# jinlinyi/PerspectiveFields

Hardware: NVIDIA H100
Metric: images/sec at 640x480 (Paramnet-360Cities-edina), H100 vs ref CPU (higher is better)
Workload: dtype f32 via 3x bf16 split MMA, fp32 accumulate

## Files before the change

### perspectivefields_b200/csrc/gemm_tma.cuh

```cuda
#pragma once
#include <cuda.h>

#include "tc_ptx.cuh"

namespace pf {

constexpr int MODE_GEMM = 0, MODE_HALO = 1;
constexpr int kTmaThreads = 384;
constexpr int kHaloBytes = 180 * 128;

struct TmaGemmParams {
  int M;
  int B, H, W;
  int Cin;
  int N, K;
  int a_c0, a_gc;
  int c_split, a2_c0;
  int groups;
  int b_row0;
  const float* bias; int bias_mode, bias_gstride;
  int act; const float* gamma;
  const float* res;  int ldr, r_coff, r_gcoff, res_relu;
  const float* res2; int ldr2, r2_coff, r2_gcoff;
  float* C; int ldc, c_coff, c_gcoff;
  __nv_bfloat16* Shi; __nv_bfloat16* Slo; int lds, s_coff, s_gcoff, split_relu;
  const float* pred_w; const float* pred_b; float* pred_out; int pred_nc, pred_mode;
  int phase4;
};

template <int BN, int MODE, int KB, bool PP = false, int NP = 3> struct TmaCfg {
  static_assert(KB == 32 || KB == 64, "KB");
  static_assert(BN % 32 == 0 && BN <= 256, "BN");
  static_assert(!PP || MODE == MODE_GEMM, "the ping-pong schedule is a GEMM-mode schedule");
  static_assert(NP == 1 || NP == 3, "NP");
  static constexpr int kPlanes = NP == 3 ? 2 : 1;
  static constexpr int kTileM = PP ? 64 : 128;
  static constexpr int kBPlane = BN * KB * 2;
  static constexpr int kAPlane = kTileM * KB * 2;
  static constexpr int kStage = (MODE == MODE_GEMM ? kPlanes * kAPlane : 0) + kPlanes * kBPlane;
  static constexpr int kABuf = kPlanes * kHtPlaneBytes;
  static constexpr int kAccPitch = 68;
  static constexpr int kAccStage = 2 * 64 * kAccPitch * 4;
  static constexpr int kBudget = 225 * 1024 - kAccStage - (MODE == MODE_HALO ? 2 * kABuf : 0);
  static constexpr int kStagesRaw = kBudget / kStage;
  static constexpr int kStages = kStagesRaw > 16 ? 16 : kStagesRaw;
  static constexpr int kSmemBytes = (MODE == MODE_HALO ? 2 * kABuf : 0) + kStages * kStage + kAccStage + 512 + 1024;
  static_assert(kStages >= 2, "ring too shallow");
  static_assert(kSmemBytes <= 227 * 1024, "shared memory per block");
};

__device__ __forceinline__ void mbar_expect_tx(uint32_t bar, uint32_t bytes) {
  asm volatile("mbarrier.arrive.expect_tx.shared::cta.b64 _, [%0], %1;\n" ::"r"(bar), "r"(bytes) : "memory");
}
__device__ __forceinline__ void tma_load_2d(uint32_t dst, const CUtensorMap* map, uint32_t bar, int c0, int c1) {
  asm volatile("cp.async.bulk.tensor.2d.shared::cluster.global.mbarrier::complete_tx::bytes [%0], [%1, {%3, %4}], [%2];\n"
               ::"r"(dst), "l"(reinterpret_cast<uint64_t>(map)), "r"(bar), "r"(c0), "r"(c1) : "memory");
}
__device__ __forceinline__ void tma_load_4d(uint32_t dst, const CUtensorMap* map, uint32_t bar, int c0, int c1, int c2, int c3) {
  asm volatile("cp.async.bulk.tensor.4d.shared::cluster.global.mbarrier::complete_tx::bytes [%0], [%1, {%3, %4, %5, %6}], [%2];\n"
               ::"r"(dst), "l"(reinterpret_cast<uint64_t>(map)), "r"(bar), "r"(c0), "r"(c1), "r"(c2), "r"(c3) : "memory");
}
__device__ __forceinline__ void tma_prefetch_desc(const CUtensorMap* map) {
  asm volatile("prefetch.tensormap [%0];\n" ::"l"(reinterpret_cast<uint64_t>(map)) : "memory");
}

struct TmaMaps {
  CUtensorMap a_hi, a_lo, a2_hi, a2_lo, b_hi, b_lo;
};

template <int BN, int MODE, int KB, bool PP = false, int NP = 3>
__global__ void __launch_bounds__(kTmaThreads, 1) gemm_tma_kernel(const __grid_constant__ TmaMaps maps, const TmaGemmParams p, int tiles_x, int tiles_y) {
  using Cfg = TmaCfg<BN, MODE, KB, PP, NP>;
  constexpr bool kLo = NP == 3;
  constexpr int NS = Cfg::kStages;
  constexpr int SPC = 9 * (64 / KB);
  constexpr int kConsumerWarps = PP ? 4 : 8;
  extern __shared__ unsigned char smem_dyn[];
  const uint32_t raw = smem_u32(smem_dyn);
  const uint32_t sbase = (raw + 1023u) & ~1023u;
  unsigned char* sm = smem_dyn + (sbase - raw);
  const uint32_t a_base = sbase;
  const uint32_t ring = sbase + (MODE == MODE_HALO ? 2 * Cfg::kABuf : 0);
  const uint32_t acc_base = ring + NS * Cfg::kStage;
  const uint32_t bars = acc_base + Cfg::kAccStage;
  auto full_b = [&](int s) { return bars + 8u * s; };
  auto empty_b = [&](int s) { return bars + 8u * (NS + s); };
  auto full_a = [&](int i) { return bars + 8u * (2 * NS + i); };
  auto empty_a = [&](int i) { return bars + 8u * (2 * NS + 2 + i); };
  auto order_b = [&](int w) { return bars + 8u * (2 * NS + 4 + w); };

  const int tid = threadIdx.x, lane = tid & 31, warp = tid >> 5;
  const int n_tiles = cdiv(p.N, BN);
  const int m_tiles = MODE == MODE_GEMM ? cdiv(p.M, Cfg::kTileM) : p.B * tiles_x * tiles_y;
  const int total_tiles = m_tiles * n_tiles * p.groups;
  const int nchunks = MODE == MODE_HALO ? p.Cin / 64 : 0;
  const int nk = MODE == MODE_GEMM ? p.K / KB : nchunks * SPC;
  const bool b_resident = MODE == MODE_HALO && nchunks == 1 && SPC <= NS;

  if (tid == 0) {
    tma_prefetch_desc(&maps.a_hi); tma_prefetch_desc(&maps.b_hi);
    if (kLo) { tma_prefetch_desc(&maps.a_lo); tma_prefetch_desc(&maps.b_lo); }
    for (int s = 0; s < NS; ++s) { mbar_init(full_b(s), 1); mbar_init(empty_b(s), kConsumerWarps); }
    for (int i = 0; i < 2; ++i) { mbar_init(full_a(i), 1); mbar_init(empty_a(i), kConsumerWarps); mbar_init(order_b(i), 4); }
    fence_mbar_init();
  }
  __syncthreads();
  pdl_wait();
  pdl_launch();

  auto decode = [&](int tile, int& mt, int& g, int& n0) {
    n0 = (tile % n_tiles) * BN;
    tile /= n_tiles;
    g = tile % p.groups;
    mt = tile / p.groups;
  };

  if (warp < 4) {
    asm volatile("setmaxnreg.dec.sync.aligned.u32 40;\n");
    if (warp == 0 && lane == 0) {
      int it = 0;
      for (int tile = blockIdx.x; tile < total_tiles; tile += gridDim.x) {
        int mt, g, n0;
        decode(tile, mt, g, n0);
        const int brow = p.b_row0 + g * p.N + n0;
        if (b_resident && it > 0) break;
        for (int kc = 0; kc < nk; ++kc, ++it) {
          const int s = it % NS;
          mbar_wait(empty_b(s), ((it / NS) & 1) ^ 1);
          mbar_expect_tx(full_b(s), Cfg::kStage);
          const uint32_t st = ring + s * Cfg::kStage;
          int kcol;
          if (MODE == MODE_GEMM) {
            kcol = kc * KB;
            tma_load_2d(st, &maps.a_hi, full_b(s), p.a_c0 + g * p.a_gc + kcol, mt * Cfg::kTileM);
            if (kLo) tma_load_2d(st + Cfg::kAPlane, &maps.a_lo, full_b(s), p.a_c0 + g * p.a_gc + kcol, mt * Cfg::kTileM);
          } else {
            const int c = kc / SPC, u = kc - c * SPC;
            kcol = KB == 32 ? (u >> 1) * p.Cin + c * 64 + (u & 1) * 32 : u * p.Cin + c * 64;
          }
          const uint32_t bdst = st + (MODE == MODE_GEMM ? Cfg::kPlanes * Cfg::kAPlane : 0);
          tma_load_2d(bdst, &maps.b_hi, full_b(s), kcol, brow);
          if (kLo) tma_load_2d(bdst + Cfg::kBPlane, &maps.b_lo, full_b(s), kcol, brow);
        }
      }
    } else if (MODE == MODE_HALO && warp == 1 && lane == 0) {
      int ita = 0;
      for (int tile = blockIdx.x; tile < total_tiles; tile += gridDim.x) {
        int mt, g, n0;
        decode(tile, mt, g, n0);
        const int tx = mt % tiles_x, ty = (mt / tiles_x) % tiles_y, bimg = mt / (tiles_x * tiles_y);
        for (int c = 0; c < nchunks; ++c, ++ita) {
          const int buf = ita & 1;
          mbar_wait(empty_a(buf), ((ita >> 1) & 1) ^ 1);
          mbar_expect_tx(full_a(buf), Cfg::kPlanes * kHaloBytes);
          const uint32_t dst = a_base + buf * Cfg::kABuf;
          const int ci = c * 64;
          if (p.c_split > 0 && ci >= p.c_split) {
            tma_load_4d(dst, &maps.a2_hi, full_a(buf), p.a2_c0 + ci - p.c_split, tx * kHtTileW - 1, ty * kHtTileH - 1, bimg);
            if (kLo) tma_load_4d(dst + kHtPlaneBytes, &maps.a2_lo, full_a(buf), p.a2_c0 + ci - p.c_split, tx * kHtTileW - 1, ty * kHtTileH - 1, bimg);
          } else {
            tma_load_4d(dst, &maps.a_hi, full_a(buf), p.a_c0 + g * p.a_gc + ci, tx * kHtTileW - 1, ty * kHtTileH - 1, bimg);
            if (kLo) tma_load_4d(dst + kHtPlaneBytes, &maps.a_lo, full_a(buf), p.a_c0 + g * p.a_gc + ci, tx * kHtTileW - 1, ty * kHtTileH - 1, bimg);
          }
        }
      }
    }
    return;
  }

  asm volatile("setmaxnreg.inc.sync.aligned.u32 232;\n");
  const int wg = (warp >> 2) - 1;
  const int wt = tid & 127;
  float* stage = reinterpret_cast<float*>(sm + (acc_base - sbase)) + wg * 64 * Cfg::kAccPitch;
  const int erow = wt & 63, eh = wt >> 6;
  const int r = PP ? erow : wg * 64 + erow;
  constexpr int kTileStep = PP ? 2 : 1;
  float acc[BN / 2];
  int it = 0, ita = 0;
  for (int tl = PP ? wg : 0, tile = blockIdx.x + tl * gridDim.x; tile < total_tiles; tile += kTileStep * gridDim.x, tl += kTileStep) {
    int mt, g, n0;
    decode(tile, mt, g, n0);
    if (PP) {
      it = tl * nk;
      if (tl > 0) mbar_wait(order_b(wg ^ 1), ((tl - 1) >> 1) & 1);
    }
    int prev_s = -1, prev_buf = -1;
    fence_regs(acc);
    for (int kc = 0; kc < nk; ++kc, ++it) {
      const int s = it % NS;
      uint32_t a_hi, a_lo;
      bool chunk_end = false;
      int buf = 0;
      if (MODE == MODE_HALO) {
        const int c = kc / SPC, u = kc - c * SPC;
        const int tap = KB == 32 ? (u >> 1) : u, ky = tap / 3, kx = tap - ky * 3;
        buf = ita & 1;
        if (u == 0) mbar_wait(full_a(buf), (ita >> 1) & 1);
        a_hi = a_base + buf * Cfg::kABuf + ((ky + 8 * wg) * kHtHaloW + kx) * 128 + (KB == 32 ? (u & 1) * 64 : 0);
        a_lo = a_hi + kHtPlaneBytes;
        chunk_end = u == SPC - 1;
      } else {
        a_hi = ring + s * Cfg::kStage + (PP ? 0 : wg * 64 * KB * 2);
        a_lo = a_hi + Cfg::kAPlane;
      }
      const int sb = b_resident ? kc : s;
      if (!b_resident || tl == 0) mbar_wait(full_b(sb), b_resident ? 0 : ((it / NS) & 1));
      const uint32_t b_hi = ring + sb * Cfg::kStage + (MODE == MODE_GEMM ? Cfg::kPlanes * Cfg::kAPlane : 0);
      const uint64_t dah = MODE == MODE_HALO ? ht_a_desc(a_hi) : wgmma_tile_desc<KB>(a_hi);
      const uint64_t dbh = wgmma_tile_desc<KB>(b_hi);
      wgmma_fence();
      if (kLo) {
        const uint64_t dal = MODE == MODE_HALO ? ht_a_desc(a_lo) : wgmma_tile_desc<KB>(a_lo);
        const uint64_t dbl = wgmma_tile_desc<KB>(b_hi + Cfg::kBPlane);
#pragma unroll
        for (int kk = 0; kk < KB / 16; ++kk) {
          const uint32_t first = (kc | kk) ? 1u : 0u;
          wgmma_bf16<BN>(acc, dal + 2 * kk, dbh + 2 * kk, first);
          wgmma_bf16<BN>(acc, dah + 2 * kk, dbl + 2 * kk, 1u);
          wgmma_bf16<BN>(acc, dah + 2 * kk, dbh + 2 * kk, 1u);
        }
      } else {
#pragma unroll
        for (int kk = 0; kk < KB / 16; ++kk) wgmma_bf16<BN>(acc, dah + 2 * kk, dbh + 2 * kk, (kc | kk) ? 1u : 0u);
      }
      wgmma_commit();
      wgmma_wait<1>();
      if (lane == 0 && prev_s >= 0) {
        if (!b_resident) mbar_arrive(empty_b(prev_s));
        if (MODE == MODE_HALO && prev_buf >= 0) mbar_arrive(empty_a(prev_buf));
      }
      prev_s = s;
      prev_buf = chunk_end ? buf : -1;
      if (MODE == MODE_HALO && chunk_end) ++ita;
    }
    if (PP && lane == 0) mbar_arrive(order_b(wg));
    wgmma_wait<0>();
    fence_regs(acc);
    if (lane == 0 && prev_s >= 0) {
      if (!b_resident) mbar_arrive(empty_b(prev_s));
      if (MODE == MODE_HALO && prev_buf >= 0) mbar_arrive(empty_a(prev_buf));
    }

    long long m;
    bool valid;
    int cls_off = 0;
    int bimg = 0, oy = 0, ox = 0;
    if (MODE == MODE_GEMM) {
      m = (long long)mt * Cfg::kTileM + r;
      valid = m < p.M;
    } else {
      const int tx = mt % tiles_x, ty = (mt / tiles_x) % tiles_y;
      bimg = mt / (tiles_x * tiles_y);
      oy = ty * kHtTileH + (r >> 3); ox = tx * kHtTileW + (r & 7);
      valid = oy < p.H && ox < p.W;
      m = ((long long)bimg * p.H + oy) * p.W + ox;
      if (p.bias_mode == 2) {
        const int ry = oy == 0 ? 0 : (oy == p.H - 1 ? 2 : 1);
        const int rx = ox == 0 ? 0 : (ox == p.W - 1 ? 2 : 1);
        cls_off = (ry * 3 + rx) * p.N;
      }
    }
    const float* __restrict__ bias = p.bias ? p.bias + (long long)g * p.bias_gstride : nullptr;
    const int frow = (wt >> 5) * 16 + (lane >> 2), fcol = 2 * (lane & 3);
#pragma unroll
    for (int rd = 0; rd < (BN + 63) / 64; ++rd) {
      named_bar_sync(1 + wg, 128);
#pragma unroll
      for (int jb = 0; jb < 8; ++jb) {
        const int cb = rd * 8 + jb;
        if (cb < BN / 8) {
          float* d0 = stage + frow * Cfg::kAccPitch + jb * 8 + fcol;
          *reinterpret_cast<float2*>(d0) = make_float2(acc[4 * cb], acc[4 * cb + 1]);
          *reinterpret_cast<float2*>(d0 + 8 * Cfg::kAccPitch) = make_float2(acc[4 * cb + 2], acc[4 * cb + 3]);
        }
      }
      named_bar_sync(1 + wg, 128);
      const int ch = 2 * rd + eh;
      const bool ph4 = MODE == MODE_HALO && BN == 128 && p.phase4;
      const bool staged_split = p.Shi && !ph4;
      float o[32];
      if (ch < BN / 32) {
        const int nb = n0 + ch * 32;
        const long long mo = ph4 ? ((long long)bimg * 2 * p.H + 2 * oy + (ch >> 1)) * (2 * p.W) + 2 * ox + (ch & 1) : m;
        const int nbo = ph4 ? 0 : nb;
        const bool chunk_ok = nb < p.N;
        const float* srow = stage + erow * Cfg::kAccPitch + eh * 32;
#pragma unroll
        for (int j = 0; j < 32; j += 4) {
          const float4 t = *reinterpret_cast<const float4*>(srow + j);
          o[j] = t.x; o[j + 1] = t.y; o[j + 2] = t.z; o[j + 3] = t.w;
        }
        if (valid && chunk_ok) {
          if (p.bias_mode) {
#pragma unroll
            for (int j = 0; j < 32; j += 4) {
              const float4 bv = __ldg(reinterpret_cast<const float4*>(bias + cls_off + nb + j));
              o[j] += bv.x; o[j + 1] += bv.y; o[j + 2] += bv.z; o[j + 3] += bv.w;
            }
          }
          if (p.act == 1) {
#pragma unroll
            for (int j = 0; j < 32; ++j) o[j] = fmaxf(o[j], 0.f);
          } else if (p.act == 2) {
#pragma unroll
            for (int j = 0; j < 32; ++j) o[j] = gelu_erf(o[j]);
          }
          if (p.gamma) {
#pragma unroll
            for (int j = 0; j < 32; j += 4) {
              const float4 gv = __ldg(reinterpret_cast<const float4*>(p.gamma + nb + j));
              o[j] *= gv.x; o[j + 1] *= gv.y; o[j + 2] *= gv.z; o[j + 3] *= gv.w;
            }
          }
          if (p.res) {
            const float* rp = p.res + m * p.ldr + p.r_coff + g * p.r_gcoff + nb;
#pragma unroll
            for (int j = 0; j < 32; j += 4) {
              float4 rv = *reinterpret_cast<const float4*>(rp + j);
              if (p.res_relu) { rv.x = fmaxf(rv.x, 0.f); rv.y = fmaxf(rv.y, 0.f); rv.z = fmaxf(rv.z, 0.f); rv.w = fmaxf(rv.w, 0.f); }
              o[j] += rv.x; o[j + 1] += rv.y; o[j + 2] += rv.z; o[j + 3] += rv.w;
            }
          }
          if (p.res2) {
            const float* rp = p.res2 + m * p.ldr2 + p.r2_coff + g * p.r2_gcoff + nb;
#pragma unroll
            for (int j = 0; j < 32; j += 4) {
              const float4 rv = *reinterpret_cast<const float4*>(rp + j);
              o[j] += rv.x; o[j + 1] += rv.y; o[j + 2] += rv.z; o[j + 3] += rv.w;
            }
          }
          if (MODE == MODE_HALO && (BN == 32 || BN == 128) && p.pred_w) {
            float v0 = __ldg(p.pred_b), v1 = p.pred_nc > 1 ? __ldg(p.pred_b + 1) : 0.f;
#pragma unroll
            for (int j = 0; j < 32; j += 4) {
              const float4 w0 = __ldg(reinterpret_cast<const float4*>(p.pred_w + j));
              v0 = fmaf(o[j], w0.x, v0); v0 = fmaf(o[j + 1], w0.y, v0); v0 = fmaf(o[j + 2], w0.z, v0); v0 = fmaf(o[j + 3], w0.w, v0);
              if (p.pred_nc > 1) {
                const float4 w1 = __ldg(reinterpret_cast<const float4*>(p.pred_w + 32 + j));
                v1 = fmaf(o[j], w1.x, v1); v1 = fmaf(o[j + 1], w1.y, v1); v1 = fmaf(o[j + 2], w1.z, v1); v1 = fmaf(o[j + 3], w1.w, v1);
              }
            }
            const long long HWl = (long long)p.H * p.W * (ph4 ? 4 : 1);
            const long long bi = mo / HWl, pix = mo - bi * HWl;
            float* po = p.pred_out + bi * p.pred_nc * HWl + pix;
            if (p.pred_mode == 1) {
              const float nrm = fmaxf(sqrtf(v0 * v0 + v1 * v1), 1e-12f);
              po[0] = v0 / nrm; po[HWl] = v1 / nrm;
            } else {
              po[0] = fminf(fmaxf(v0, -1.f), 1.f);
            }
          }
        }
        if (chunk_ok && (p.C || (p.Shi && !staged_split))) {
          const bool odd = lane & 1;
          const bool valid_p = __shfl_xor_sync(0xffffffffu, (int)valid, 1) != 0;
          const long long mo_p = mo + (odd ? -1 : 1) * (ph4 ? 2 : 1);
          const long long moA = odd ? mo_p : mo, moB = odd ? mo : mo_p;
          const bool vA = odd ? valid_p : valid, vB = odd ? valid : valid_p;
          if (p.C) {
            float* cA = p.C + moA * p.ldc + p.c_coff + g * p.c_gcoff + nbo + (odd ? 4 : 0);
            float* cB = p.C + moB * p.ldc + p.c_coff + g * p.c_gcoff + nbo + (odd ? 4 : 0);
#pragma unroll
            for (int t = 0; t < 4; ++t) {
              float k[4], rr[4];
#pragma unroll
              for (int e = 0; e < 4; ++e) {
                k[e] = odd ? o[8 * t + 4 + e] : o[8 * t + e];
                rr[e] = __shfl_xor_sync(0xffffffffu, odd ? o[8 * t + e] : o[8 * t + 4 + e], 1);
              }
              if (vA) *reinterpret_cast<float4*>(cA + 8 * t) = odd ? make_float4(rr[0], rr[1], rr[2], rr[3]) : make_float4(k[0], k[1], k[2], k[3]);
              if (vB) *reinterpret_cast<float4*>(cB + 8 * t) = odd ? make_float4(k[0], k[1], k[2], k[3]) : make_float4(rr[0], rr[1], rr[2], rr[3]);
            }
          }
          if (p.Shi && !staged_split) {
            const long long sA = moA * p.lds + p.s_coff + g * p.s_gcoff + nbo + (odd ? 8 : 0);
            const long long sB = moB * p.lds + p.s_coff + g * p.s_gcoff + nbo + (odd ? 8 : 0);
#pragma unroll
            for (int t = 0; t < 2; ++t) {
              float k[8], rr[8];
#pragma unroll
              for (int e = 0; e < 8; ++e) {
                const float mine = odd ? o[16 * t + 8 + e] : o[16 * t + e], give = odd ? o[16 * t + e] : o[16 * t + 8 + e];
                k[e] = p.split_relu ? fmaxf(mine, 0.f) : mine;
                rr[e] = __shfl_xor_sync(0xffffffffu, p.split_relu ? fmaxf(give, 0.f) : give, 1);
              }
              uint4 kh, kl, rh, rl;
              split_bf16x2(k[0], k[1], kh.x, kl.x); split_bf16x2(k[2], k[3], kh.y, kl.y);
              split_bf16x2(k[4], k[5], kh.z, kl.z); split_bf16x2(k[6], k[7], kh.w, kl.w);
              split_bf16x2(rr[0], rr[1], rh.x, rl.x); split_bf16x2(rr[2], rr[3], rh.y, rl.y);
              split_bf16x2(rr[4], rr[5], rh.z, rl.z); split_bf16x2(rr[6], rr[7], rh.w, rl.w);
              if (vA) {
                *reinterpret_cast<uint4*>(p.Shi + sA + 16 * t) = odd ? rh : kh;
                *reinterpret_cast<uint4*>(p.Slo + sA + 16 * t) = odd ? rl : kl;
              }
              if (vB) {
                *reinterpret_cast<uint4*>(p.Shi + sB + 16 * t) = odd ? kh : rh;
                *reinterpret_cast<uint4*>(p.Slo + sB + 16 * t) = odd ? kl : rl;
              }
            }
          }
        }
      }
      if (staged_split) {
        named_bar_sync(1 + wg, 128);
        unsigned char* sS = reinterpret_cast<unsigned char*>(stage);
        if (ch < BN / 32) {
#pragma unroll
          for (int t = 0; t < 4; ++t) {
            uint4 h, l;
            float k[8];
#pragma unroll
            for (int e = 0; e < 8; ++e) k[e] = p.split_relu ? fmaxf(o[8 * t + e], 0.f) : o[8 * t + e];
            split_bf16x2(k[0], k[1], h.x, l.x); split_bf16x2(k[2], k[3], h.y, l.y);
            split_bf16x2(k[4], k[5], h.z, l.z); split_bf16x2(k[6], k[7], h.w, l.w);
            const int off = erow * 128 + (((eh * 4 + t) ^ (erow & 7)) << 4);
            *reinterpret_cast<uint4*>(sS + off) = h;
            *reinterpret_cast<uint4*>(sS + 64 * 128 + off) = l;
          }
        }
        named_bar_sync(1 + wg, 128);
#pragma unroll
        for (int i = wt; i < 2 * 64 * 8; i += 128) {
          const int lo_plane = i >> 9, rr = (i >> 3) & 63, pc = i & 7;
          const int col = rd * 64 + pc * 8;
          if (col >= BN || n0 + col >= p.N) continue;
          long long mr;
          bool vr;
          if (MODE == MODE_GEMM) {
            mr = (long long)mt * Cfg::kTileM + (PP ? 0 : wg * 64) + rr;
            vr = mr < p.M;
          } else {
            const int rt = wg * 64 + rr, tx = mt % tiles_x, ty = (mt / tiles_x) % tiles_y;
            const int py = ty * kHtTileH + (rt >> 3), px = tx * kHtTileW + (rt & 7);
            vr = py < p.H && px < p.W;
            mr = ((long long)bimg * p.H + py) * p.W + px;
          }
          if (!vr) continue;
          const uint4 v = *reinterpret_cast<const uint4*>(sS + lo_plane * 64 * 128 + rr * 128 + ((pc ^ (rr & 7)) << 4));
          *reinterpret_cast<uint4*>((lo_plane ? p.Slo : p.Shi) + mr * p.lds + p.s_coff + g * p.s_gcoff + n0 + col) = v;
        }
      }
    }
  }
}

}
```

### perspectivefields_b200/csrc/pf_b200.cu

```cuda
#include "../../include/pf_b200.h"

#include <cuda_runtime.h>
#include <nvtx3/nvToolsExt.h>

#include <atomic>
#include <cctype>
#include <cmath>
#include <cstdarg>
#include <cstdio>
#include <cstdlib>
#include <cstring>
#include <map>
#include <mutex>
#include <string>
#include <functional>
#include <unordered_map>
#include <vector>

#include "common.cuh"
#include "tma_host.cuh"
#include "attention_mma.cuh"
#include "layers.cuh"
#include "prepost.cuh"
#include "pano.cuh"
#include "comm.cuh"
#include "jpeg.cuh"

using namespace pf;

static thread_local std::string g_err;
static std::atomic<long long> g_launches{0};

static int fail(int code, const char* fmt, ...) {
  char buf[1024];
  va_list ap;
  va_start(ap, fmt);
  vsnprintf(buf, sizeof(buf), fmt, ap);
  va_end(ap);
  g_err = buf;
  return code;
}
#define CU(expr)                                                                                    \
  do {                                                                                              \
    cudaError_t e__ = (expr);                                                                       \
    if (e__ != cudaSuccess) return fail(PF_ERR_CUDA, "%s: %s (%s:%d)", #expr, cudaGetErrorString(e__), __FILE__, __LINE__); \
  } while (0)
static char g_crumb[96] = "";
static bool sync_debug() {
  static int v = -1;
  if (v < 0) v = getenv("PF_SYNC_DEBUG") ? 1 : 0;
  return v == 1;
}
struct KernelProf {
  bool on = false;
  cudaStream_t st = nullptr;
  std::vector<cudaEvent_t> pool;
  size_t used = 0;
  struct Rec { const char* expr; cudaEvent_t a, b; };
  std::vector<Rec> recs;
  cudaEvent_t next() { return used < pool.size() ? pool[used++] : nullptr; }
};
static thread_local KernelProf* tl_kp = nullptr;
#define LAUNCHED(expr)                                                                              \
  do {                                                                                              \
    KernelProf* kp__ = tl_kp;                                                                       \
    cudaEvent_t ka__ = (kp__ && kp__->on) ? kp__->next() : nullptr;                                 \
    if (ka__) cudaEventRecord(ka__, kp__->st);                                                      \
    cudaError_t e__ = (expr);                                                                       \
    g_launches.fetch_add(1, std::memory_order_relaxed);                                             \
    if (ka__) {                                                                                     \
      cudaEvent_t kb__ = kp__->next();                                                              \
      if (kb__) { cudaEventRecord(kb__, kp__->st); kp__->recs.push_back({#expr, ka__, kb__}); }     \
    }                                                                                               \
    if (e__ == cudaSuccess && sync_debug()) e__ = cudaDeviceSynchronize();                          \
    if (e__ != cudaSuccess) return fail(PF_ERR_CUDA, "%s: %s (%s:%d, after tap '%s')", #expr, cudaGetErrorString(e__), __FILE__, __LINE__, g_crumb); \
  } while (0)
struct NvtxRange {
  explicit NvtxRange(const char* name) { nvtxRangePushA(name); }
  ~NvtxRange() { nvtxRangePop(); }
};
#define TRY(expr)                \
  do {                           \
    int r__ = (expr);            \
    if (r__ != PF_OK) return r__; \
  } while (0)

static const int kMitDims[4] = {64, 128, 320, 512};
static const int kMitHeads[4] = {1, 2, 5, 8};
static const int kMitDepths[4] = {3, 4, 18, 3};
static const int kMitSr[4] = {8, 4, 2, 1};
static const int kCnxDims[4] = {96, 192, 384, 768};
static const int kCnxDepths[4] = {3, 3, 9, 3};

struct WeightRef { const void* p; long long numel; int dtype; };
struct GemmW { const __nv_bfloat16* hi = nullptr; const __nv_bfloat16* lo = nullptr; const float* b = nullptr; };
struct LnW { const float* w = nullptr; const float* b = nullptr; };

struct MitBlockW { LnW ln1, srln, ln2; GemmW q, sr, kv, proj, fc1, fc2; const float* dw_w; const float* dw_b; };
struct CnxBlockW { const float* dw_w; const float* dw_b; LnW ln; GemmW pw1, pw2; const float* gamma; };

struct Arena {
  char* base = nullptr;
  long long cap = 0, off = 0, peak = 0;
  bool dry = false, keep = false;
  void* alloc(long long bytes) {
    off = (off + 255) & ~255LL;
    void* p = dry ? nullptr : base + off;
    off += bytes;
    if (off > peak) peak = off;
    return p;
  }
  float* f(long long n) { return (float*)alloc(n * 4); }
  long long mark() const { return off; }
  void release(long long m) { if (!keep) off = m; }
};

struct pf_engine {
  int device = 0;
  pf_model_desc desc{};
  int net_h = kNet, net_w = kNet;
  bool finalized = false;
  std::unordered_map<std::string, WeightRef> weights;
  const float *embed1_w, *embed1_b, *llenc_w, *llenc_b;
  LnW embed_ln[4], stage_norm[4];
  GemmW embed[4];
  GemmW embed1g, llencg;
  std::vector<MitBlockW> blocks[4];
  GemmW proc[4];
  GemmW rcu[4][2][2];
  GemmW conv0, conv1;
  GemmW conv1p;
  const float *conv1f_w, *conv1f_b;
  bool use_fork = false;
  cudaStream_t side = nullptr;
  cudaEvent_t ev_fork = nullptr, ev_join = nullptr;
  bool use_dwln = false;
  bool use_pdl = true;
  bool decode_only = false;
  bool use_attn_split = true;
  bool use_phase = true;
  const float *pred_g_w, *pred_g_b, *pred_l_w, *pred_l_b;
  const float *pn_stem_w, *pn_stem_b;
  LnW pn_stem_ln, pn_ds_ln[4], pn_norm;
  GemmW pn_ds[4];
  std::vector<CnxBlockW> pn_blocks[4];
  const float *pn_head_w, *pn_head_b;
  struct DevTable { int ksize; int* bounds; int* coeffs; };
  std::map<std::pair<int, int>, DevTable> tables;
  char* table_dev = nullptr;
  char* table_host = nullptr;
  long long table_off = 0;
  KernelProf kp;
  struct MapKey {
    const void* base; long long d0, d1, d2; int kind, box, kb;
    bool operator==(const MapKey& o) const { return base == o.base && d0 == o.d0 && d1 == o.d1 && d2 == o.d2 && kind == o.kind && box == o.box && kb == o.kb; }
  };
  struct MapKeyHash {
    size_t operator()(const MapKey& k) const {
      size_t h = std::hash<const void*>()(k.base);
      for (long long v : {k.d0, k.d1, k.d2, (long long)k.kind, (long long)k.box, (long long)k.kb}) h = h * 1000003u ^ std::hash<long long>()(v);
      return h;
    }
  };
  std::unordered_map<MapKey, CUtensorMap, MapKeyHash> map_cache;
  bool use_stem_tc = true;
  bool use_attn_mma = true;
  bool bf16 = false;
  int sm_count = 132;
  bool profile = false;
  struct ProfRec { cudaEvent_t a, b; double flops; int cfg; int M, N, K, KH, stride, groups, Cin; };
  std::vector<ProfRec> prof;
  std::vector<cudaEvent_t> ev_pool;
  bool debug = false;
  std::vector<std::pair<std::string, std::pair<const float*, long long>>> taps;
};

static int get_w(pf_engine* e, const std::string& name, int dtype, long long numel, const void** out) {
  auto it = e->weights.find(name);
  if (it == e->weights.end()) return fail(PF_ERR_WEIGHT, "missing weight '%s'", name.c_str());
  if (it->second.dtype != dtype) return fail(PF_ERR_WEIGHT, "weight '%s': wrong dtype", name.c_str());
  if (it->second.numel != numel) return fail(PF_ERR_WEIGHT, "weight '%s': numel %lld, expected %lld", name.c_str(), it->second.numel, numel);
  *out = it->second.p;
  return PF_OK;
}
static int get_f(pf_engine* e, const std::string& n, long long numel, const float** out) { return get_w(e, n, PF_F32, numel, (const void**)out); }
static int get_gemm(pf_engine* e, const std::string& n, long long N, long long K, long long nbias, GemmW* g, int groups = 1) {
  TRY(get_w(e, n + ".whi", PF_BF16, groups * N * K, (const void**)&g->hi));
  TRY(get_w(e, n + ".wlo", PF_BF16, groups * N * K, (const void**)&g->lo));
  TRY(get_f(e, n + ".b", groups * nbias, &g->b));
  return PF_OK;
}
static int get_ln(pf_engine* e, const std::string& n, int C, LnW* l) {
  TRY(get_f(e, n + ".w", C, &l->w));
  TRY(get_f(e, n + ".b", C, &l->b));
  return PF_OK;
}

static int resolve_weights(pf_engine* e) {
  char nm[128];
  TRY(get_f(e, "embed1.w", 147 * 64, &e->embed1_w));
  TRY(get_f(e, "embed1.b", 64, &e->embed1_b));
  TRY(get_f(e, "llenc.w", 147 * 64, &e->llenc_w));
  TRY(get_f(e, "llenc.b", 64, &e->llenc_b));
  TRY(get_gemm(e, "embed1g", 64, 160, 64, &e->embed1g));
  TRY(get_gemm(e, "llencg", 64, 160, 64, &e->llencg));
  for (int s = 0; s < 4; ++s) {
    const int C = kMitDims[s];
    snprintf(nm, sizeof nm, "embed%d.ln", s + 1);
    TRY(get_ln(e, nm, C, &e->embed_ln[s]));
    if (s > 0) {
      snprintf(nm, sizeof nm, "embed%d", s + 1);
      TRY(get_gemm(e, nm, C, 9LL * kMitDims[s - 1], C, &e->embed[s]));
    }
    e->blocks[s].resize(kMitDepths[s]);
    for (int i = 0; i < kMitDepths[s]; ++i) {
      MitBlockW& b = e->blocks[s][i];
      char p[64];
      snprintf(p, sizeof p, "s%d.b%d.", s + 1, i);
      std::string P(p);
      TRY(get_ln(e, P + "ln1", C, &b.ln1));
      TRY(get_gemm(e, P + "q", C, C, C, &b.q));
      if (kMitSr[s] > 1) {
        TRY(get_gemm(e, P + "sr", C, (long long)kMitSr[s] * kMitSr[s] * C, C, &b.sr));
        TRY(get_ln(e, P + "srln", C, &b.srln));
      }
      TRY(get_gemm(e, P + "kv", 2 * C, C, 2 * C, &b.kv));
      TRY(get_gemm(e, P + "proj", C, C, C, &b.proj));
      TRY(get_ln(e, P + "ln2", C, &b.ln2));
      TRY(get_gemm(e, P + "fc1", 4 * C, C, 4 * C, &b.fc1));
      TRY(get_f(e, P + "dw.w", 9LL * 4 * C, &b.dw_w));
      TRY(get_f(e, P + "dw.b", 4 * C, &b.dw_b));
      TRY(get_gemm(e, P + "fc2", C, 4 * C, C, &b.fc2));
    }
    snprintf(nm, sizeof nm, "s%d.norm", s + 1);
    TRY(get_ln(e, nm, C, &e->stage_norm[s]));
  }
  for (int l = 0; l < 4; ++l) {
    snprintf(nm, sizeof nm, "head.proc%d", l + 1);
    TRY(get_gemm(e, nm, 512, 9LL * kMitDims[l], 9 * 512, &e->proc[l]));
  }
  for (int f = 0; f < 4; ++f)
    for (int u = 0; u < 2; ++u) {
      if (f == 3 && u == 0) continue;
      for (int c = 0; c < 2; ++c) {
        snprintf(nm, sizeof nm, "head.f%d.u%d.c%d", f + 1, u + 1, c + 1);
        TRY(get_gemm(e, nm, 256, 2304, 256, &e->rcu[f][u][c], 2));
      }
    }
  TRY(get_gemm(e, "head.conv0", 64, 9 * 320, 64, &e->conv0, 2));
  TRY(get_gemm(e, "head.conv1", 32, 9 * 64, 32, &e->conv1, 2));
  TRY(get_gemm(e, "head.conv1p", 128, 9 * 64, 128, &e->conv1p, 2));
  TRY(get_f(e, "head.conv1f.w", 2LL * 9 * 64 * 32, &e->conv1f_w));
  TRY(get_f(e, "head.conv1f.b", 64, &e->conv1f_b));
  TRY(get_f(e, "head.pred_g.w", 32LL * e->desc.gravity_classes, &e->pred_g_w));
  TRY(get_f(e, "head.pred_g.b", e->desc.gravity_classes, &e->pred_g_b));
  TRY(get_f(e, "head.pred_l.w", 32LL * e->desc.latitude_classes, &e->pred_l_w));
  TRY(get_f(e, "head.pred_l.b", e->desc.latitude_classes, &e->pred_l_b));
  if (e->desc.param_net != PF_PARAM_NONE) {
    TRY(get_f(e, "pn.stem.w", 48 * 96, &e->pn_stem_w));
    TRY(get_f(e, "pn.stem.b", 96, &e->pn_stem_b));
    TRY(get_ln(e, "pn.stem.ln", 96, &e->pn_stem_ln));
    for (int k = 1; k < 4; ++k) {
      snprintf(nm, sizeof nm, "pn.ds%d.ln", k);
      TRY(get_ln(e, nm, kCnxDims[k - 1], &e->pn_ds_ln[k]));
      snprintf(nm, sizeof nm, "pn.ds%d", k);
      TRY(get_gemm(e, nm, kCnxDims[k], 4LL * kCnxDims[k - 1], kCnxDims[k], &e->pn_ds[k]));
    }
    for (int s = 0; s < 4; ++s) {
      const int C = kCnxDims[s];
      e->pn_blocks[s].resize(kCnxDepths[s]);
      for (int j = 0; j < kCnxDepths[s]; ++j) {
        CnxBlockW& b = e->pn_blocks[s][j];
        char p[64];
        snprintf(p, sizeof p, "pn.s%d.b%d.", s, j);
        std::string P(p);
        TRY(get_f(e, P + "dw.w", 49LL * C, &b.dw_w));
        TRY(get_f(e, P + "dw.b", C, &b.dw_b));
        TRY(get_ln(e, P + "ln", C, &b.ln));
        TRY(get_gemm(e, P + "pw1", 4 * C, C, 4 * C, &b.pw1));
        TRY(get_gemm(e, P + "pw2", C, 4 * C, C, &b.pw2));
        TRY(get_f(e, P + "gamma", C, &b.gamma));
      }
    }
    TRY(get_ln(e, "pn.norm", 768, &e->pn_norm));
    TRY(get_f(e, "pn.head.w", 5 * 768, &e->pn_head_w));
    TRY(get_f(e, "pn.head.b", 5, &e->pn_head_b));
  }
  return PF_OK;
}

struct Fwd {
  pf_engine* e;
  Arena ar;
  cudaStream_t st;
  bool dry;
  int n;

  int tap(const char* name, const float* p, long long numel) {
    if (!e->debug) return PF_OK;
    float* cp = ar.f(numel);
    if (dry) return PF_OK;
    snprintf(g_crumb, sizeof g_crumb, "%s", name);
    if (sync_debug()) fprintf(stderr, "[pf tap] %s cp=%p (+%lld of cap %lld) p=%p numel=%lld\n", name, (void*)cp, (long long)((char*)cp - ar.base), ar.cap, (const void*)p, numel);
    CU(cudaMemcpyAsync(cp, p, numel * 4, cudaMemcpyDeviceToDevice, st));
    if (sync_debug()) CU(cudaDeviceSynchronize());
    e->taps.push_back({name, {cp, numel}});
    return PF_OK;
  }
  int tapf(const float* p, long long numel, const char* fmt, ...) {
    if (!e->debug) return PF_OK;
    char buf[96];
    va_list ap;
    va_start(ap, fmt);
    vsnprintf(buf, sizeof buf, fmt, ap);
    va_end(ap);
    return tap(buf, p, numel);
  }

  SplitT salloc(long long pixels, int ld) {
    SplitT t;
    t.hi = (__nv_bfloat16*)ar.alloc(pixels * ld * 2);
    t.lo = (__nv_bfloat16*)ar.alloc(pixels * ld * 2);
    t.ld = ld;
    return t;
  }
  int tap_split(const char* name, const SplitT& t, long long numel) {
    if (!e->debug) return PF_OK;
    float* cp = ar.f(numel);
    if (dry) return PF_OK;
    snprintf(g_crumb, sizeof g_crumb, "%s", name);
    LAUNCHED((merge_split_kernel<<<(unsigned)cdivl(numel, 256), 256, 0, st>>>(t.hi, t.lo, cp, numel), cudaGetLastError()));
    e->taps.push_back({name, {cp, numel}});
    return PF_OK;
  }
  static cudaError_t gemm_tma_gemm_mode(const TmaMaps& maps, const TmaGemmParams& p, int bn, int kb, bool pp, int np, int sms, cudaStream_t st, const PredTail* pred) {
    return gemm_tma_launch(MODE_GEMM, maps, p, bn, kb, pp, np, sms, st, pred);
  }
  static cudaError_t gemm_tma_halo_mode(const TmaMaps& maps, const TmaGemmParams& p, int bn, int kb, bool pp, int np, int sms, cudaStream_t st, const PredTail* pred) {
    return gemm_tma_launch(MODE_HALO, maps, p, bn, kb, pp, np, sms, st, pred);
  }
  int np() const { return e->bf16 ? 1 : 3; }
  int force_bn = 0, force_kb = 0;
  int force_sched = 0;
  int picked_bn = 0, picked_kb = 0, picked_sched = 0;
  int pick_tile(int mode, const TmaGemmParams& p, const PredTail* pred, int& bn, int& kb, bool& pp) {
    tma_pick_tile(mode, p.M, p.N, p.K, e->sm_count, bn, kb);
    if (force_bn) { bn = force_bn; kb = tma_pick_kb(bn, p.K, mode); }
    if (force_kb) kb = force_kb;
    pp = mode == MODE_GEMM && (force_sched ? force_sched == 2 : tma_pick_pingpong(p.M, p.N, p.K, bn, e->sm_count));
    if (const char* msg = gemm_tma_check(mode, p, bn, kb, pred != nullptr, pp, np())) return fail(PF_ERR_ARG, "TMA engine, %s (bn %d, kb %d): %s", mode == MODE_GEMM ? "GEMM mode" : "halo mode", bn, kb, msg);
    picked_bn = bn; picked_kb = kb; picked_sched = mode == MODE_GEMM ? (pp ? 2 : 1) : 0;
    return PF_OK;
  }
  int launch_tma(int mode, const TmaMaps& maps, const TmaGemmParams& p, int bn, int kb, bool pp, const PredTail* pred = nullptr) {
    if (e->profile) {
      pf_engine::ProfRec r{};
      for (cudaEvent_t* ev : {&r.a, &r.b}) {
        if (e->ev_pool.empty()) { CU(cudaEventCreate(ev)); }
        else { *ev = e->ev_pool.back(); e->ev_pool.pop_back(); }
      }
      const double Mrows = mode == MODE_GEMM ? (double)p.M : (double)p.B * p.H * p.W;
      r.flops = 2.0 * Mrows * (double)p.N * (double)p.K * (double)p.groups;
      r.cfg = mode == MODE_GEMM ? 5 : 6;
      r.M = (int)Mrows; r.N = p.N; r.K = p.K; r.KH = mode == MODE_GEMM ? 1 : 3; r.stride = 1; r.groups = p.groups; r.Cin = p.Cin;
      CU(cudaEventRecord(r.a, st));
      if (mode == MODE_GEMM) LAUNCHED(gemm_tma_gemm_mode(maps, p, bn, kb, pp, np(), e->sm_count, st, pred));
      else LAUNCHED(gemm_tma_halo_mode(maps, p, bn, kb, pp, np(), e->sm_count, st, pred));
      CU(cudaEventRecord(r.b, st));
      e->prof.push_back(r);
      return PF_OK;
    }
    if (mode == MODE_GEMM) LAUNCHED(gemm_tma_gemm_mode(maps, p, bn, kb, pp, np(), e->sm_count, st, pred));
    else LAUNCHED(gemm_tma_halo_mode(maps, p, bn, kb, pp, np(), e->sm_count, st, pred));
    return PF_OK;
  }
  struct Epi {
    float* C = nullptr; int ldc = 0, c_coff = 0, c_gcoff = 0;
    SplitT S; int s_coff = 0, s_gcoff = 0, split_relu = 0;
    int act = 0; const float* gamma = nullptr;
    const float* res = nullptr; int ldr = 0, r_coff = 0, r_gcoff = 0, res_relu = 0;
    const float* res2 = nullptr; int ldr2 = 0, r2_coff = 0, r2_gcoff = 0;
    int bias_mode = 1;
    int phase4 = 0;
  };
  static void fill_epi(TmaGemmParams& p, const GemmW& w, const Epi& o, int bias_gstride) {
    p.bias = w.b; p.bias_mode = w.b ? o.bias_mode : 0; p.bias_gstride = bias_gstride;
    p.act = o.act; p.gamma = o.gamma;
    p.res = o.res; p.ldr = o.ldr; p.r_coff = o.r_coff; p.r_gcoff = o.r_gcoff; p.res_relu = o.res_relu;
    p.res2 = o.res2; p.ldr2 = o.ldr2; p.r2_coff = o.r2_coff; p.r2_gcoff = o.r2_gcoff;
    p.C = o.C; p.ldc = o.ldc; p.c_coff = o.c_coff; p.c_gcoff = o.c_gcoff;
    p.Shi = o.S.hi; p.Slo = o.S.lo; p.lds = o.S.ld; p.s_coff = o.s_coff; p.s_gcoff = o.s_gcoff; p.split_relu = o.split_relu;
    p.phase4 = o.phase4;
  }
  template <class F>
  const char* cached_map(CUtensorMap* out, const pf_engine::MapKey& key, F&& make) {
    auto it = e->map_cache.find(key);
    if (it != e->map_cache.end()) { *out = it->second; return nullptr; }
    const char* msg = make(out);
    if (!msg) {
      if (e->map_cache.size() > 20000) e->map_cache.clear();
      e->map_cache.emplace(key, *out);
    }
    return msg;
  }
  const char* map2d(CUtensorMap* m, const void* base, long long cols, long long rows, long long ld, int box_rows, int kb) {
    return cached_map(m, pf_engine::MapKey{base, cols, rows, ld, 0, box_rows, kb}, [&](CUtensorMap* o) { return tma_map_2d(o, base, cols, rows, ld, box_rows, kb); });
  }
  const char* map_halo(CUtensorMap* m, const void* base, int B, int H, int W, int ld) {
    return cached_map(m, pf_engine::MapKey{base, ((long long)B << 32) | (unsigned)H, W, ld, 3, 0, 0}, [&](CUtensorMap* o) { return tma_map_halo(o, base, B, H, W, ld); });
  }
  int tgemm(const SplitT& A, long long M, int K, int a_c0, const GemmW& w, int N, const Epi& o) {
    if (dry) return PF_OK;
    if (K % 32 || N % 32 || A.ld % 8) return fail(PF_ERR_ARG, "tgemm: K/N must be multiples of 32");
    if (o.res2 || o.bias_mode == 2) return fail(PF_ERR_ARG, "tgemm: second residual / border-class bias are halo-mode features");
    TmaGemmParams p{};
    p.M = (int)M; p.Cin = K; p.N = N; p.K = K; p.a_c0 = a_c0; p.groups = 1;
    fill_epi(p, w, o, 0);
    TmaMaps maps{};
    int bn, kb;
    bool pp;
    TRY(pick_tile(MODE_GEMM, p, nullptr, bn, kb, pp));
    const char* msg = nullptr;
    const int a_rows = pp ? 64 : 128;
    if (!msg) msg = map2d(&maps.a_hi, A.hi, A.ld, M, A.ld, a_rows, kb);
    if (!msg) msg = map2d(&maps.a_lo, A.lo, A.ld, M, A.ld, a_rows, kb);
    if (!msg) msg = map2d(&maps.b_hi, w.hi, K, N, K, bn, kb);
    if (!msg) msg = map2d(&maps.b_lo, w.lo, K, N, K, bn, kb);
    if (msg) return fail(PF_ERR_CUDA, "%s", msg);
    maps.a2_hi = maps.a_hi; maps.a2_lo = maps.a_lo;
    return launch_tma(MODE_GEMM, maps, p, bn, kb, pp);
  }
  int thalo(const SplitT& A, int a_c0, int a_gc, const SplitT* A2, int c_split, int a2_c0, int B, int H, int W, int Cin, const GemmW& w, int N,
            int groups, int bias_gstride, const Epi& o, const PredTail* pred = nullptr) {
    if (dry) return PF_OK;
    if (Cin % 64 || N % 32 || (A2 && c_split % 64)) return fail(PF_ERR_ARG, "thalo: Cin must be a multiple of 64, N of 32");
    if (w.b && o.bias_mode == 2 && (H < 2 || W < 2)) return fail(PF_ERR_ARG, "thalo: border-class bias needs H, W >= 2 (got %dx%d)", H, W);
    TmaGemmParams p{};
    p.B = B; p.H = H; p.W = W; p.Cin = Cin; p.N = N; p.K = 9 * Cin; p.a_c0 = a_c0; p.a_gc = a_gc; p.groups = groups;
    p.c_split = A2 ? c_split : 0; p.a2_c0 = a2_c0;
    fill_epi(p, w, o, bias_gstride);
    TmaMaps maps{};
    int bn, kb;
    bool pp;
    TRY(pick_tile(MODE_HALO, p, pred, bn, kb, pp));
    const char* msg = nullptr;
    if (!msg) msg = map_halo(&maps.a_hi, A.hi, B, H, W, A.ld);
    if (!msg) msg = map_halo(&maps.a_lo, A.lo, B, H, W, A.ld);
    if (A2) {
      if (!msg) msg = map_halo(&maps.a2_hi, A2->hi, B, H, W, A2->ld);
      if (!msg) msg = map_halo(&maps.a2_lo, A2->lo, B, H, W, A2->ld);
    } else { maps.a2_hi = maps.a_hi; maps.a2_lo = maps.a_lo; }
    if (!msg) msg = map2d(&maps.b_hi, w.hi, p.K, (long long)groups * N, p.K, bn, kb);
    if (!msg) msg = map2d(&maps.b_lo, w.lo, p.K, (long long)groups * N, p.K, bn, kb);
    if (msg) return fail(PF_ERR_CUDA, "%s", msg);
    return launch_tma(MODE_HALO, maps, p, bn, kb, pp, pred);
  }
  int tconv_gather(const SplitT& A, int B, int H, int W, int Cin, int KH, int stride, int pad, const GemmW& w, int N, const Epi& o) {
    const int OH = (H + 2 * pad - KH) / stride + 1, OW = (W + 2 * pad - KH) / stride + 1;
    const long long M = (long long)B * OH * OW;
    const int K = KH * KH * Cin;
    const long long m = ar.mark();
    SplitT col = salloc(M, K);
    if (!dry) {
      if (Cin % 8) return fail(PF_ERR_ARG, "tconv_gather: Cin %% 8");
      LAUNCHED(launch_pdl(im2col_split_kernel, dim3(ew_grid(M * K / 8)), dim3(256), 0, st, A.hi, A.lo, A.ld, col.hi, col.lo, B, H, W, Cin, OH, OW, KH, stride, pad));
    }
    int r = tgemm(col, M, K, 0, w, N, o);
    ar.release(m);
    return r;
  }
  int ln_split(const float* x, const SplitT& y, long long rows, int C, const LnW& w, float eps, float* yf = nullptr) {
    if (dry) return PF_OK;
    LAUNCHED(layernorm_launch(x, yf, rows, C, w.w, w.b, eps, st, y));
    return PF_OK;
  }
  int ln_split_patch(const float* x, const SplitT& y, const SplitT& patch, long long rows, int C, const LnW& w, float eps, int RH, int RW, int sr) {
    if (dry) return PF_OK;
    LAUNCHED(layernorm_launch(x, nullptr, rows, C, w.w, w.b, eps, st, y, patch, RH, RW, sr));
    return PF_OK;
  }
  int ln(const float* x, float* y, long long rows, int C, const LnW& w, float eps) {
    if (dry) return PF_OK;
    LAUNCHED(layernorm_launch(x, y, rows, C, w.w, w.b, eps, st));
    return PF_OK;
  }
};

constexpr long long kTableSlabBytes = 8LL << 20;
static int get_table(pf_engine* e, int in_size, int out_size, pf_engine::DevTable* out, cudaStream_t st) {
  auto it = e->tables.find({in_size, out_size});
  if (it == e->tables.end()) {
    ResampleTable t = make_resample_table(in_size, out_size);
    const long long nb = (long long)t.bounds.size() * sizeof(int), nc = (long long)t.coeffs.size() * sizeof(int);
    const long long need = ((nb + 255) & ~255LL) + ((nc + 255) & ~255LL);
    if (need > kTableSlabBytes) return fail(PF_ERR_ARG, "image axis of %d pixels is too long for the resize tables", in_size);
    if (e->table_off + need > kTableSlabBytes) {
      CU(cudaStreamSynchronize(st));
      e->tables.clear();
      e->table_off = 0;
    }
    pf_engine::DevTable d{};
    d.ksize = t.ksize;
    const long long o0 = e->table_off, o1 = o0 + ((nb + 255) & ~255LL);
    memcpy(e->table_host + o0, t.bounds.data(), nb);
    memcpy(e->table_host + o1, t.coeffs.data(), nc);
    d.bounds = (int*)(e->table_dev + o0);
    d.coeffs = (int*)(e->table_dev + o1);
    CU(cudaMemcpyAsync(e->table_dev + o0, e->table_host + o0, need, cudaMemcpyHostToDevice, st));
    e->table_off += need;
    it = e->tables.emplace(std::make_pair(in_size, out_size), d).first;
  }
  *out = it->second;
  return PF_OK;
}

static int pre_rows_needed(int H, int OH) {
  const double scale = (double)H / OH;
  const double support = scale < 1.0 ? 1.0 : scale;
  return (int)(kPreRows * scale) + 2 * (int)ceil(support) + 3;
}
static int pre_max_smem_rows(int OW) { return kPreSmemBytes / (OW * 3); }

static int fwd_preprocess(Fwd& F, const pf_batch* bt, float*& x0, PreImage*& d_pre, PostImage*& d_post) {
  pf_engine* e = F.e;
  const pf_model_desc& D = e->desc;
  const int n = F.n;
  const bool dry = F.dry;
  cudaStream_t st = F.st;
  Arena& ar = F.ar;
  const int NH = e->net_h, NW = e->net_w;
  const int max_rows = pre_max_smem_rows(NW);
  x0 = ar.f((long long)n * NH * NW * 4);
  d_pre = (PreImage*)ar.alloc((long long)n * sizeof(PreImage));
  d_post = (PostImage*)ar.alloc((long long)n * sizeof(PostImage));
  if (!dry) {
    if (bt->images_u8) {
      std::vector<PreImage> pre(n);
      int max_h = 1;
      for (int i = 0; i < n; ++i) {
        const int H = bt->height[i], W = bt->width[i];
        if (H < 1 || W < 1) return fail(PF_ERR_ARG, "image %d has size %dx%d", i, H, W);
        pf_engine::DevTable tx, ty;
        TRY(get_table(e, W, NW, &tx, st));
        TRY(get_table(e, H, NH, &ty, st));
        if (ty.ksize + 1 > max_rows) return fail(PF_ERR_ARG, "image %d is too tall (%d rows) for the resize kernel", i, H);
        pre[i] = PreImage{bt->image_offset[i], H, W, tx.ksize, ty.ksize, tx.bounds, tx.coeffs, ty.bounds, ty.coeffs};
        if (H > max_h) max_h = H;
      }
      CU(cudaMemcpyAsync(d_pre, pre.data(), n * sizeof(PreImage), cudaMemcpyHostToDevice, st));
      int rows = pre_rows_needed(max_h, NH);
      if (rows > max_rows) rows = max_rows;
      const int smem = rows * NW * 3;
      LAUNCHED((preprocess_kernel<<<dim3(NH / kPreRows, n), NW, smem, st>>>(bt->images_u8, d_pre, x0, D.pixel_mean[0], D.pixel_mean[1],
                                                                           D.pixel_mean[2], D.pixel_std[0], D.pixel_std[1], D.pixel_std[2], rows, NH, NW),
                cudaGetLastError()));
    } else {
      const long long total = (long long)n * NH * NW;
      LAUNCHED((normalize_chw_kernel<<<(unsigned)cdivl(total, 256), 256, 0, st>>>(bt->images_chw, x0, n, NH, NW, D.pixel_mean[0], D.pixel_mean[1],
                                                                                 D.pixel_mean[2], D.pixel_std[0], D.pixel_std[1], D.pixel_std[2]),
                cudaGetLastError()));
    }
  }
  return PF_OK;
}

static int launch_postprocess(const float* vec, const float* lat, int n, int SH, int SW, const int32_t* height, const int32_t* width, const int64_t* g_off,
                              const int64_t* l_off, float* g_out, float* l_out, int lat_is_sin, PostImage* d_post, cudaStream_t st) {
  std::vector<PostImage> post(n);
  long long total = 0;
  int max_h = 1, max_wp = 4;
  for (int i = 0; i < n; ++i) {
    if (height[i] < 1 || width[i] < 1) return fail(PF_ERR_ARG, "image %d has size %dx%d", i, height[i], width[i]);
    post[i] = PostImage{height[i], width[i], g_off[i], l_off[i], total};
    total += (long long)height[i] * width[i];
    if (height[i] > max_h) max_h = height[i];
    const int wp = (width[i] + 3) / 4 * 4;
    if (wp <= kPostMaxW && wp > max_wp) max_wp = wp;
  }
  CU(cudaMemcpyAsync(d_post, post.data(), n * sizeof(PostImage), cudaMemcpyHostToDevice, st));
  const int smem = post_smem_bytes(SW, max_wp);
  LAUNCHED((postprocess_kernel<<<dim3((unsigned)cdiv(max_h, kPostBand), (unsigned)n), kPostThreads, smem, st>>>(vec, lat, d_post, g_out, l_out, lat_is_sin, SH, SW),
            cudaGetLastError()));
  return PF_OK;
}

static int fwd_tails_post(Fwd& F, const pf_batch* bt, const float* conv1_out, PostImage* d_post, bool pred_done = false) {
  pf_engine* e = F.e;
  const pf_model_desc& D = e->desc;
  const int n = F.n;
  const bool dry = F.dry;
  cudaStream_t st = F.st;
  Arena& ar = F.ar;
  const int HW = e->net_h * e->net_w;
  const bool cls_g = D.gravity_classes != 2, cls_l = D.latitude_classes != 1;
  const bool fused_decode = e->decode_only && (cls_g || cls_l);
  if (e->decode_only && cls_g != cls_l) return fail(PF_ERR_ARG, "decode_only needs both heads to be classification heads");
  const float* vec = dry ? nullptr : bt->pred_gravity;
  const float* lat = dry ? nullptr : bt->pred_latitude;
  if (e->debug) {
    float* rg = ar.f((long long)n * D.gravity_classes * HW);
    float* rl = ar.f((long long)n * D.latitude_classes * HW);
    if (!dry) {
      const unsigned grid = (unsigned)cdivl((long long)n * HW, 128);
      LAUNCHED((pred_tail_kernel<<<grid, 128, D.gravity_classes * 33 * 4, st>>>(conv1_out, 64, 0, e->pred_g_w, e->pred_g_b, rg, n, HW, D.gravity_classes, 0), cudaGetLastError()));
      LAUNCHED((pred_tail_kernel<<<grid, 128, D.latitude_classes * 33 * 4, st>>>(conv1_out, 64, 32, e->pred_l_w, e->pred_l_b, rl, n, HW, D.latitude_classes, 0), cudaGetLastError()));
    }
    TRY(F.tap("head.raw_g", rg, (long long)n * D.gravity_classes * HW));
    TRY(F.tap("head.raw_l", rl, (long long)n * D.latitude_classes * HW));
  }
  if (fused_decode) {
    if (!dry) {
      const unsigned grid = ew_grid((long long)n * HW * 4);
      LAUNCHED((pred_argmax_decode_kernel<<<grid, 256, D.gravity_classes * 37 * 4, st>>>(conv1_out, 64, 0, e->pred_g_w, e->pred_g_b, bt->pred_gravity, n, HW,
                                                                                      D.gravity_classes, 1), cudaGetLastError()));
      LAUNCHED((pred_argmax_decode_kernel<<<grid, 256, D.latitude_classes * 37 * 4, st>>>(conv1_out, 64, 32, e->pred_l_w, e->pred_l_b, bt->pred_latitude, n, HW,
                                                                                       D.latitude_classes, 0), cudaGetLastError()));
    }
  } else {
    if (!dry && !pred_done) {
      const unsigned grid = (unsigned)cdivl((long long)n * HW, 128);
      LAUNCHED((pred_tail_kernel<<<grid, 128, D.gravity_classes * 33 * 4, st>>>(conv1_out, 64, 0, e->pred_g_w, e->pred_g_b, bt->pred_gravity, n, HW,
                                                                             D.gravity_classes, D.gravity_classes == 2 ? 1 : 0), cudaGetLastError()));
      LAUNCHED((pred_tail_kernel<<<grid, 128, D.latitude_classes * 33 * 4, st>>>(conv1_out, 64, 32, e->pred_l_w, e->pred_l_b, bt->pred_latitude, n, HW,
                                                                              D.latitude_classes, D.latitude_classes == 1 ? 2 : 0), cudaGetLastError()));
    }
    if (cls_g) {
      float* dv = ar.f((long long)n * 2 * HW);
      if (!dry) LAUNCHED((argmax_decode_kernel<<<(unsigned)cdivl((long long)n * HW, 256), 256, 0, st>>>(bt->pred_gravity, dv, n, HW, D.gravity_classes, 1), cudaGetLastError()));
      vec = dv;
    }
    if (cls_l) {
      float* dl = ar.f((long long)n * HW);
      if (!dry) LAUNCHED((argmax_decode_kernel<<<(unsigned)cdivl((long long)n * HW, 256), 256, 0, st>>>(bt->pred_latitude, dl, n, HW, D.latitude_classes, 0), cudaGetLastError()));
      lat = dl;
    }
  }
  if (!dry)
    TRY(launch_postprocess(vec, lat, n, e->net_h, e->net_w, bt->height, bt->width, bt->gravity_original_offset, bt->latitude_original_offset, bt->gravity_original,
                           bt->latitude_original, cls_l ? 0 : 1, d_post, st));
  return PF_OK;
}

static int run_forward_tma(Fwd& F, const pf_batch* bt) {
  pf_engine* e = F.e;
  const pf_model_desc& D = e->desc;
  const int n = F.n;
  const bool dry = F.dry;
  cudaStream_t st = F.st;
  Arena& ar = F.ar;
  using Epi = Fwd::Epi;
  const int NH = e->net_h, NW = e->net_w;
  int RH[4], RW[4];
  for (int s = 0; s < 4; ++s) { RH[s] = NH >> (s + 2); RW[s] = NW >> (s + 2); }
  const int nkv = RH[3] * RW[3];
  if ((NH != kNet || NW != kNet) && (!e->use_attn_mma || !e->use_attn_split || !e->use_stem_tc || !e->use_phase))
    return fail(PF_ERR_ARG, "options attn_mma / attn_split / stem_tc / phase_conv1 = 0 (reference paths of the 320 x 320 graph) need a 320 x 320 "
                            "working size; this engine runs at %d x %d", NH, NW);

  float* x0; PreImage* d_pre; PostImage* d_post;
  {
    NvtxRange r_("pf:preprocess");
    TRY(fwd_preprocess(F, bt, x0, d_pre, d_post));
  }
  TRY(F.tap("pre", x0, (long long)n * NH * NW * 4));

  NvtxRange* sect = new NvtxRange("pf:ll_enc");
  struct SectGuard { NvtxRange*& p; ~SectGuard() { delete p; } } sect_guard{sect};
  auto section = [&](const char* name) { delete sect; sect = nullptr; sect = new NvtxRange(name); };
  SplitT cfeat[4];
  for (int s = 0; s < 4; ++s) cfeat[s] = F.salloc((long long)n * RH[s] * RW[s], kMitDims[s]);
  const int LH = NH / 2, LW = NW / 2;
  SplitT ll = F.salloc((long long)n * LH * LW, 64);
  if (e->use_stem_tc) {
    const long long m = ar.mark();
    const long long M = (long long)n * LH * LW;
    SplitT col = F.salloc(M, 160);
    if (!dry) LAUNCHED(launch_pdl(stem_gather_kernel, dim3(ew_grid(stem_gather_threads(n, LH, LW))), dim3(256), 0, st, x0, col.hi, col.lo, n, LH, LW, 2, NH, NW));
    Epi o; o.S = ll; o.act = 1;
    TRY(F.tgemm(col, M, 160, 0, e->llencg, 64, o));
    ar.release(m);
  } else if (!dry) {
    LAUNCHED((stem_conv_launch<7, 7, 2, 3, 64>(x0, 4, n, kNet, kNet, e->llenc_w, e->llenc_b, nullptr, 1, st, ll)));
  }
  TRY(F.tap_split("ll", ll, (long long)n * LH * LW * 64));

  for (int s = 0; s < 4; ++s) {
    { char nm[32]; snprintf(nm, sizeof nm, "pf:mit.stage%d", s + 1); section(nm); }
    const int C = kMitDims[s], N = RH[s] * RW[s], heads = kMitHeads[s], sr = kMitSr[s];
    const long long rows = (long long)n * N;
    const long long m = ar.mark();
    float* x = ar.f(rows * C);
    float* tf = ar.f(rows * C);
    SplitT t1 = F.salloc(rows, C);
    SplitT t1p;
    if (sr > 1) t1p = F.salloc((long long)n * nkv, sr * sr * C);
    SplitT q = F.salloc(rows, C);
    SplitT a = F.salloc(rows, C);
    float* t2f = ar.f((long long)n * nkv * C);
    SplitT t2 = F.salloc((long long)n * nkv, C);
    SplitT kv = F.salloc((long long)n * nkv, 2 * C);
    const bool qkv_split = e->use_attn_mma && e->use_attn_split;
    float* qf = qkv_split ? nullptr : ar.f(rows * C);
    float* kvf = qkv_split ? nullptr : ar.f((long long)n * nkv * 2 * C);
    float* h1 = ar.f(rows * 4 * C);
    SplitT h2 = F.salloc(rows, 4 * C);
    if (s == 0 && e->use_stem_tc) {
      const long long mm = ar.mark();
      SplitT col = F.salloc(rows, 160);
      if (!dry) LAUNCHED(launch_pdl(stem_gather_kernel, dim3(ew_grid(stem_gather_threads(n, RH[0], RW[0]))), dim3(256), 0, st, x0, col.hi, col.lo, n, RH[0], RW[0], 4, NH, NW));
      Epi o; o.C = tf; o.ldc = C;
      TRY(F.tgemm(col, rows, 160, 0, e->embed1g, 64, o));
      ar.release(mm);
    } else if (s == 0) {
      if (!dry) LAUNCHED((stem_conv_launch<7, 7, 4, 3, 64>(x0, 4, n, kNet, kNet, e->embed1_w, e->embed1_b, tf, 0, st)));
    } else {
      Epi o; o.C = tf; o.ldc = C;
      TRY(F.tconv_gather(cfeat[s - 1], n, RH[s - 1], RW[s - 1], kMitDims[s - 1], 3, 2, 1, e->embed[s], C, o));
    }
    TRY(F.ln(tf, x, rows, C, e->embed_ln[s], 1e-5f));
    TRY(F.tapf(x, rows * C, "mit.s%d.embed", s + 1));
    for (int i = 0; i < kMitDepths[s]; ++i) {
      const MitBlockW& b = e->blocks[s][i];
      if (sr > 1) TRY(F.ln_split_patch(x, t1, t1p, rows, C, b.ln1, 1e-6f, RH[s], RW[s], sr));
      else TRY(F.ln_split(x, t1, rows, C, b.ln1, 1e-6f));
      Epi oq, okv;
      if (qkv_split) { oq.S = q; okv.S = kv; } else { oq.C = qf; oq.ldc = C; okv.C = kvf; okv.ldc = 2 * C; }
      const bool fork = !dry && sr > 1 && e->use_fork && e->side && !e->kp.on && !e->profile && !sync_debug() && !e->debug;
      if (fork) {
        CU(cudaEventRecord(e->ev_fork, st));
        CU(cudaStreamWaitEvent(e->side, e->ev_fork, 0));
        F.st = e->side;
      }
      if (sr > 1) {
        { Epi o; o.C = t2f; o.ldc = C; TRY(F.tgemm(t1p, (long long)n * nkv, sr * sr * C, 0, b.sr, C, o)); }
        TRY(F.ln_split(t2f, t2, (long long)n * nkv, C, b.srln, 1e-5f));
        TRY(F.tgemm(t2, (long long)n * nkv, C, 0, b.kv, 2 * C, okv));
      }
      if (fork) {
        CU(cudaEventRecord(e->ev_join, e->side));
        F.st = st;
      }
      TRY(F.tgemm(t1, rows, C, 0, b.q, C, oq));
      if (fork) CU(cudaStreamWaitEvent(st, e->ev_join, 0));
      if (sr > 1) {
      } else {
        TRY(F.tgemm(t1, rows, C, 0, b.kv, 2 * C, okv));
      }
      if (!dry) {
        if (qkv_split) LAUNCHED(attention_mma_launch(nullptr, nullptr, nullptr, n, N, C, heads, st, a, q, kv, F.np(), nkv));
        else if (e->use_attn_mma) LAUNCHED(attention_mma_launch(qf, kvf, nullptr, n, N, C, heads, st, a, SplitT(), SplitT(), F.np()));
        else LAUNCHED(attention_launch(qf, kvf, nullptr, n, N, C, heads, st, a));
      }
      { Epi o; o.C = x; o.ldc = C; o.res = x; o.ldr = C; TRY(F.tgemm(a, rows, C, 0, b.proj, C, o)); }
      TRY(F.tapf(x, rows * C, "mit.s%d.b%d.attn", s + 1, i));
      TRY(F.ln_split(x, t1, rows, C, b.ln2, 1e-6f));
      { Epi o; o.C = h1; o.ldc = 4 * C; TRY(F.tgemm(t1, rows, C, 0, b.fc1, 4 * C, o)); }
      if (!dry) LAUNCHED(launch_pdl(dwconv3x3_gelu_kernel, dim3(ew_grid((long long)n * ((RH[s] + 1) / 2) * ((RW[s] + PF_DW3_PX - 1) / PF_DW3_PX) * C)), dim3(256), 0, st, h1, nullptr, n, RH[s], RW[s], 4 * C, b.dw_w, b.dw_b, h2.hi, h2.lo));
      { Epi o; o.C = x; o.ldc = C; o.res = x; o.ldr = C; TRY(F.tgemm(h2, rows, 4 * C, 0, b.fc2, C, o)); }
      TRY(F.tapf(x, rows * C, "mit.s%d.b%d", s + 1, i));
    }
    TRY(F.ln_split(x, cfeat[s], rows, C, e->stage_norm[s], 1e-6f));
    { char nm[32]; snprintf(nm, sizeof nm, "mit.c%d", s + 1); TRY(F.tap_split(nm, cfeat[s], rows * C)); }
    ar.release(m);
  }

  float* conv1_out = ar.f((long long)n * NH * NW * 64);
  bool fuse_pred = false;
  {
    const long long m = ar.mark();
    float* fused = nullptr;
    SplitT fused_s;
    for (int lvl = 4; lvl >= 1; --lvl) {
      { char nm[32]; snprintf(nm, sizeof nm, "pf:heads.level%d", lvl); section(nm); }
      const int rh = RH[lvl - 1], rw = RW[lvl - 1], Cin = kMitDims[lvl - 1];
      const long long px = (long long)n * rh * rw;
      float* t = ar.f(px * 512);
      SplitT rt = F.salloc(px, 512);
      SplitT u = F.salloc(px, 512);
      float* v = ar.f(px * 512);
      SplitT rv = F.salloc(px, 512);
      float* w2 = ar.f(px * 512);
      {
        Epi o; o.C = t; o.ldc = 512; o.S = rt; o.split_relu = 1; o.bias_mode = 2;
        TRY(F.thalo(cfeat[lvl - 1], 0, 0, nullptr, 0, 0, n, rh, rw, Cin, e->proc[lvl - 1], 512, 1, 0, o));
        TRY(F.tapf(t, px * 512, "head.proc%d", lvl));
      }
      auto rcu = [&](const SplitT& A, const GemmW& w, Epi o) {
        o.c_gcoff = 256; o.s_gcoff = 256; o.r_gcoff = 256; o.r2_gcoff = 256;
        return F.thalo(A, 0, 256, nullptr, 0, 0, n, rh, rw, 256, w, 256, 2, 256, o);
      };
      const float* of = t;
      const SplitT* os = &rt;
      if (lvl < 4) {
        { Epi o; o.S = u; o.act = 1; TRY(rcu(rt, e->rcu[lvl - 1][0][0], o)); }
        { Epi o; o.C = v; o.ldc = 512; o.S = rv; o.split_relu = 1; o.res = t; o.ldr = 512; o.res_relu = 1; o.res2 = fused; o.ldr2 = 512;
          TRY(rcu(u, e->rcu[lvl - 1][0][1], o)); }
        of = v; os = &rv;
      }
      { Epi o; o.S = u; o.act = 1; TRY(rcu(*os, e->rcu[lvl - 1][1][0], o)); }
      { Epi o; o.C = w2; o.ldc = 512; o.res = of; o.ldr = 512; o.res_relu = 1; TRY(rcu(u, e->rcu[lvl - 1][1][1], o)); }
      if (lvl > 1) {
        float* up = ar.f(px * 4 * 512);
        if (!dry) LAUNCHED(launch_pdl(upsample2x_kernel, dim3(ew_grid(upsample2x_threads(n, rh, rw, 512))), dim3(256), 0, st, w2, 512, 0, up, 512, 0, n, rh, rw, 512, nullptr, nullptr));
        fused = up;
        TRY(F.tapf(up, px * 4 * 512, "head.fusion%d", lvl));
      } else {
        fused_s = F.salloc(px * 4, 512);
        if (!dry) LAUNCHED(launch_pdl(upsample2x_kernel, dim3(ew_grid(upsample2x_threads(n, rh, rw, 512))), dim3(256), 0, st, w2, 512, 0, nullptr, 512, 0, n, rh, rw, 512, fused_s.hi, fused_s.lo));
        TRY(F.tap_split("head.fusion1", fused_s, px * 4 * 512));
      }
    }
    section("pf:heads.fuse_convs");
    fuse_pred = D.gravity_classes == 2 && D.latitude_classes == 1;
    const bool keep_conv1 = !fuse_pred || e->debug;
    PredTail pt[2] = {{e->pred_g_w, e->pred_g_b, dry ? nullptr : bt->pred_gravity, 2, 1}, {e->pred_l_w, e->pred_l_b, dry ? nullptr : bt->pred_latitude, 1, 2}};
    if (e->use_phase) {
      SplitT c0s = F.salloc((long long)n * LH * LW, 128);
      {
        Epi o; o.S = c0s; o.s_gcoff = 64; o.act = 1;
        TRY(F.thalo(fused_s, 0, 256, &ll, 256, 0, n, LH, LW, 320, e->conv0, 64, 2, 64, o));
        TRY(F.tap_split("head.conv0", c0s, (long long)n * LH * LW * 128));
      }
      Epi o; o.ldc = 64; o.c_gcoff = 32; o.act = 1; o.phase4 = 1;
      if (keep_conv1) o.C = conv1_out;
      TRY(F.thalo(c0s, 0, 64, nullptr, 0, 0, n, LH, LW, 64, e->conv1p, 128, 2, 128, o, fuse_pred ? pt : nullptr));
      if (!dry) {
        const dim3 grid((unsigned)cdiv(conv1_ring_count(NH, NW), kRingPx), (unsigned)n);
        LAUNCHED((conv1_ring_kernel<<<grid, 256, kRingSmem, st>>>(c0s.hi, c0s.lo, LH, LW, e->conv1f_w, e->conv1f_b, keep_conv1 ? conv1_out : nullptr,
                                                                 fuse_pred ? e->pred_g_w : nullptr, e->pred_g_b, bt->pred_gravity,
                                                                 fuse_pred ? e->pred_l_w : nullptr, e->pred_l_b, bt->pred_latitude), cudaGetLastError()));
      }
    } else {
      float* c0 = ar.f((long long)n * 160 * 160 * 128);
      {
        Epi o; o.C = c0; o.ldc = 128; o.c_gcoff = 64; o.act = 1;
        TRY(F.thalo(fused_s, 0, 256, &ll, 256, 0, n, 160, 160, 320, e->conv0, 64, 2, 64, o));
        TRY(F.tap("head.conv0", c0, (long long)n * 160 * 160 * 128));
      }
      SplitT c0u = F.salloc((long long)n * kNet * kNet, 128);
      if (!dry) LAUNCHED(launch_pdl(upsample2x_kernel, dim3(ew_grid(upsample2x_threads(n, 160, 160, 128))), dim3(256), 0, st, c0, 128, 0, nullptr, 128, 0, n, 160, 160, 128, c0u.hi, c0u.lo));
      Epi o; o.ldc = 64; o.c_gcoff = 32; o.act = 1;
      if (keep_conv1) o.C = conv1_out;
      TRY(F.thalo(c0u, 0, 64, nullptr, 0, 0, n, kNet, kNet, 64, e->conv1, 32, 2, 32, o, fuse_pred ? pt : nullptr));
    }
    if (keep_conv1) TRY(F.tap("head.conv1", conv1_out, (long long)n * NH * NW * 64));
    ar.release(m);
  }
  section("pf:tails_postprocess");
  TRY(fwd_tails_post(F, bt, conv1_out, d_post, fuse_pred));

  if (D.param_net != PF_PARAM_NONE) {
    section("pf:paramnet");
    if (D.gravity_classes != 2 || D.latitude_classes != 1) return fail(PF_ERR_ARG, "ParamNet needs regression heads");
    const bool centered = D.param_net == PF_PARAM_CENTERED;
    const int SH = centered ? NH : D.param_input_size, SW = centered ? NW : D.param_input_size;
    float* pin = ar.f((long long)n * SH * SW * 4);
    if (!dry) LAUNCHED((pack_fields_kernel<<<(unsigned)cdivl((long long)n * SH * SW, 256), 256, 0, st>>>(bt->pred_gravity, bt->pred_latitude, pin, n, NH, NW, SH, SW), cudaGetLastError()));
    int rh = SH / 4, rw = SW / 4;
    float* x = ar.f((long long)n * rh * rw * 96);
    if (!dry) LAUNCHED((stem_conv_launch<4, 4, 4, 0, 96>(pin, 4, n, SH, SW, e->pn_stem_w, e->pn_stem_b, x, 0, st)));
    TRY(F.ln(x, x, (long long)n * rh * rw, 96, e->pn_stem_ln, 1e-6f));
    for (int s = 0; s < 4; ++s) {
      const int C = kCnxDims[s];
      if (s > 0) {
        const int r2h = rh / 2, r2w = rw / 2;
        SplitT y = F.salloc((long long)n * r2h * r2w, 4 * kCnxDims[s - 1]);
        TRY(F.ln_split_patch(x, SplitT(), y, (long long)n * rh * rw, kCnxDims[s - 1], e->pn_ds_ln[s], 1e-6f, rh, rw, 2));
        float* xn = ar.f((long long)n * r2h * r2w * C);
        Epi o; o.C = xn; o.ldc = C;
        TRY(F.tgemm(y, (long long)n * r2h * r2w, 4 * kCnxDims[s - 1], 0, e->pn_ds[s], C, o));
        x = xn; rh = r2h; rw = r2w;
      }
      const long long rows = (long long)n * rh * rw;
      float* yf = ar.f(rows * C);
      SplitT y = F.salloc(rows, C);
      SplitT h = F.salloc(rows, 4 * C);
      for (int j = 0; j < kCnxDepths[s]; ++j) {
        const CnxBlockW& b = e->pn_blocks[s][j];
        if (e->use_dwln) {
          if (!dry) LAUNCHED(dwconv7x7_ln_launch(x, n, rh, rw, C, b.dw_w, b.dw_b, b.ln.w, b.ln.b, 1e-6f, y, st));
        } else {
          if (!dry) LAUNCHED(launch_pdl(dwconv7x7_kernel, dim3(ew_grid((long long)n * ((rh + 1) / 2) * ((rw + PF_DW7_PX - 1) / PF_DW7_PX) * (C / 4))), dim3(256), 0, st, x, yf, n, rh, rw, C, b.dw_w, b.dw_b));
          TRY(F.ln_split(yf, y, rows, C, b.ln, 1e-6f));
        }
        { Epi o; o.S = h; o.act = 2; TRY(F.tgemm(y, rows, C, 0, b.pw1, 4 * C, o)); }
        { Epi o; o.C = x; o.ldc = C; o.res = x; o.ldr = C; o.gamma = b.gamma; TRY(F.tgemm(h, rows, 4 * C, 0, b.pw2, C, o)); }
      }
      TRY(F.tapf(x, rows * C, "cnx.s%d", s));
    }
    if (!dry) {
      if (!bt->params) return fail(PF_ERR_ARG, "params output is NULL");
      LAUNCHED((param_tail_kernel<<<n, 256, 0, st>>>(x, rh * rw, e->pn_norm.w, e->pn_norm.b, e->pn_head_w, e->pn_head_b, bt->params, D.param_net), cudaGetLastError()));
    }
  }
  return PF_OK;
}

extern "C" {

int pf_abi_version(void) { return PF_ABI_VERSION; }
const char* pf_last_error(void) { return g_err.c_str(); }
int64_t pf_kernel_launch_count(void) { return g_launches.load(); }

static int configure_device(int device) {
  static std::mutex mu;
  static std::vector<char> done;
  std::lock_guard<std::mutex> lock(mu);
  if (device < (int)done.size() && done[device]) return PF_OK;
  CU(gemm_tma_configure_device(3));
  CU(gemm_tma_configure_device(1));
  CU(attention_mma_configure_device());
  CU(cudaFuncSetAttribute(attention_kernel, cudaFuncAttributeMaxDynamicSharedMemorySize, kAttnSmem));
  CU(cudaFuncSetAttribute(conv1_ring_kernel, cudaFuncAttributeMaxDynamicSharedMemorySize, kRingSmem));
  CU(cudaFuncSetAttribute(preprocess_kernel, cudaFuncAttributeMaxDynamicSharedMemorySize, kPreSmemBytes));
  CU(cudaFuncSetAttribute(postprocess_kernel, cudaFuncAttributeMaxDynamicSharedMemorySize, kPostSmemMax));
  if (device >= (int)done.size()) done.resize(device + 1, 0);
  done[device] = 1;
  return PF_OK;
}
static int configure_current_device() {
  int dev = 0;
  CU(cudaGetDevice(&dev));
  return configure_device(dev);
}

static bool net_size_ok(int h, int w) {
  return h >= 64 && w >= 64 && h <= 640 && w <= 640 && h % 32 == 0 && w % 32 == 0 && (h / 32) * (w / 32) <= kAmMaxKeys;
}

int pf_create(int device, const pf_model_desc* desc, pf_handle* out) { return pf_create_sized(device, desc, kNet, kNet, out); }

int pf_create_sized(int device, const pf_model_desc* desc, int net_h, int net_w, pf_handle* out) {
  if (!desc || !out) return fail(PF_ERR_ARG, "pf_create: null argument");
  if (!net_size_ok(net_h, net_w))
    return fail(PF_ERR_ARG, "pf_create: working size %dx%d: height and width must be multiples of 32 in [64, 640] with (H/32)*(W/32) <= %d", net_h, net_w, kAmMaxKeys);
  if (!((desc->gravity_classes == 2 || desc->gravity_classes == 73) && (desc->latitude_classes == 1 || desc->latitude_classes == 180)))
    return fail(PF_ERR_ARG, "pf_create: unsupported head widths %d/%d", desc->gravity_classes, desc->latitude_classes);
  if (desc->param_net < 0 || desc->param_net > 2) return fail(PF_ERR_ARG, "pf_create: bad param_net");
  if (desc->param_net == PF_PARAM_UNCENTERED && (desc->param_input_size < 32 || desc->param_input_size > kNet || desc->param_input_size % 32))
    return fail(PF_ERR_ARG, "pf_create: param_input_size must be a multiple of 32 in [32, 320]");
  int count = 0;
  CU(cudaGetDeviceCount(&count));
  if (device < 0 || device >= count) return fail(PF_ERR_CUDA, "pf_create: no CUDA device %d (found %d)", device, count);
  CU(cudaSetDevice(device));
  cudaDeviceProp prop;
  CU(cudaGetDeviceProperties(&prop, device));
  if (prop.major != 9 || prop.minor != 0) return fail(PF_ERR_CUDA, "pf_create: device %d is sm_%d%d; this library is built for sm_90a only", device, prop.major, prop.minor);
  TRY(configure_device(device));
  pf_engine* e = new pf_engine();
  e->device = device;
  e->sm_count = prop.multiProcessorCount;
  e->desc = *desc;
  e->net_h = net_h;
  e->net_w = net_w;
  if (cudaMalloc(&e->table_dev, kTableSlabBytes) != cudaSuccess || cudaMallocHost(&e->table_host, kTableSlabBytes) != cudaSuccess) {
    const int r = fail(PF_ERR_CUDA, "pf_create: resize-table slab: %s", cudaGetErrorString(cudaGetLastError()));
    cudaFree(e->table_dev);
    delete e;
    return r;
  }
  if (cudaStreamCreateWithFlags(&e->side, cudaStreamNonBlocking) != cudaSuccess || cudaEventCreateWithFlags(&e->ev_fork, cudaEventDisableTiming) != cudaSuccess ||
      cudaEventCreateWithFlags(&e->ev_join, cudaEventDisableTiming) != cudaSuccess) {
    const int r = fail(PF_ERR_CUDA, "pf_create: side stream / events: %s", cudaGetErrorString(cudaGetLastError()));
    pf_destroy(e);
    return r;
  }
  *out = e;
  return PF_OK;
}

int pf_destroy(pf_handle h) {
  if (!h) return PF_OK;
  cudaSetDevice(h->device);
  if (h->side) { cudaStreamSynchronize(h->side); cudaStreamDestroy(h->side); }
  if (h->ev_fork) cudaEventDestroy(h->ev_fork);
  if (h->ev_join) cudaEventDestroy(h->ev_join);
  cudaFree(h->table_dev);
  cudaFreeHost(h->table_host);
  for (auto& r : h->prof) { cudaEventDestroy(r.a); cudaEventDestroy(r.b); }
  for (auto ev : h->ev_pool) cudaEventDestroy(ev);
  for (auto ev : h->kp.pool) cudaEventDestroy(ev);
  delete h;
  return PF_OK;
}

int pf_set_weight(pf_handle h, const char* name, const void* dev_ptr, int64_t numel, int dtype) {
  if (!h || !name || !dev_ptr) return fail(PF_ERR_ARG, "pf_set_weight: null argument");
  if (((uintptr_t)dev_ptr & 15) != 0) return fail(PF_ERR_ARG, "pf_set_weight: '%s' is not 16-byte aligned", name);
  h->weights[name] = WeightRef{dev_ptr, numel, dtype};
  h->finalized = false;
  return PF_OK;
}

int pf_finalize(pf_handle h) {
  if (!h) return fail(PF_ERR_ARG, "pf_finalize: null handle");
  TRY(resolve_weights(h));
  h->finalized = true;
  return PF_OK;
}

int64_t pf_workspace_bytes(pf_handle h, int n, int max_h) {
  if (!h || n < 1) return fail(PF_ERR_ARG, "pf_workspace_bytes: bad argument");
  Fwd F{h, Arena{}, nullptr, true, n};
  F.ar.dry = true;
  F.ar.keep = h->debug;
  (void)max_h;
  int r = run_forward_tma(F, nullptr);
  if (r != PF_OK) return r;
  return F.ar.peak + 4096;
}

int pf_forward(pf_handle h, const pf_batch* bt, void* workspace, int64_t workspace_bytes, void* stream) {
  if (!h || !bt || !workspace) return fail(PF_ERR_ARG, "pf_forward: null argument");
  if (!h->finalized) return fail(PF_ERR_WEIGHT, "pf_forward: pf_finalize has not succeeded");
  if (bt->n < 1) return fail(PF_ERR_ARG, "pf_forward: empty batch");
  if ((bt->images_u8 != nullptr) == (bt->images_chw != nullptr)) return fail(PF_ERR_ARG, "pf_forward: exactly one of images_u8 / images_chw");
  if (bt->images_u8 && !bt->image_offset) return fail(PF_ERR_ARG, "pf_forward: image_offset is NULL");
  if (!bt->height || !bt->width || !bt->pred_gravity || !bt->pred_latitude || !bt->gravity_original || !bt->latitude_original ||
      !bt->gravity_original_offset || !bt->latitude_original_offset)
    return fail(PF_ERR_ARG, "pf_forward: null input/output pointer");
  CU(cudaSetDevice(h->device));
  Fwd F{h, Arena{}, (cudaStream_t)stream, false, bt->n};
  F.ar.base = (char*)workspace;
  F.ar.cap = workspace_bytes;
  F.ar.keep = h->debug;
  {
    Fwd T{h, Arena{}, nullptr, true, bt->n};
    T.ar.dry = true; T.ar.keep = h->debug;
    TRY(run_forward_tma(T, nullptr));
    if (T.ar.peak > workspace_bytes) return fail(PF_ERR_WORKSPACE, "pf_forward: workspace %lld B < required %lld B", (long long)workspace_bytes, T.ar.peak);
  }
  if (((uintptr_t)workspace & 255) != 0) return fail(PF_ERR_ARG, "pf_forward: workspace must be 256-byte aligned");
  h->taps.clear();
  h->kp.st = (cudaStream_t)stream;
  tl_kp = &h->kp;
  pdl_enabled() = h->use_pdl && !h->kp.on && !h->profile && !sync_debug();
  const int r = run_forward_tma(F, bt);
  pdl_enabled() = false;
  tl_kp = nullptr;
  return r;
}

int pf_profile_enable(pf_handle h, int on) {
  if (!h) return fail(PF_ERR_ARG, "null handle");
  h->profile = on != 0;
  while (on > 1 && (long long)h->ev_pool.size() < 2LL * on) {
    cudaEvent_t ev;
    CU(cudaEventCreate(&ev));
    h->ev_pool.push_back(ev);
  }
  return PF_OK;
}
int pf_profile_kernels_enable(pf_handle h, int max_launches) {
  if (!h) return fail(PF_ERR_ARG, "null handle");
  CU(cudaSetDevice(h->device));
  KernelProf& kp = h->kp;
  kp.on = max_launches > 0;
  kp.used = 0;
  kp.recs.clear();
  while ((long long)kp.pool.size() < 2LL * max_launches) {
    cudaEvent_t ev;
    CU(cudaEventCreate(&ev));
    kp.pool.push_back(ev);
  }
  return PF_OK;
}
int pf_profile_kernels_read(pf_handle h, char* buf, int cap) {
  if (!h || !buf || cap < 1) return fail(PF_ERR_ARG, "pf_profile_kernels_read: bad argument");
  std::map<std::string, std::pair<int, double>> agg;
  std::vector<std::string> order;
  for (const auto& r : h->kp.recs) {
    float ms = 0.f;
    CU(cudaEventElapsedTime(&ms, r.a, r.b));
    const char* c = r.expr;
    while (*c == '(' || *c == ' ') ++c;
    const char* e = c;
    while (*e && (isalnum((unsigned char)*e) || *e == '_')) ++e;
    std::string name(c, e);
    if (name == "launch_pdl" && *e == '(') {
      c = e + 1;
      e = c;
      while (*e && (isalnum((unsigned char)*e) || *e == '_')) ++e;
      name.assign(c, e);
    }
    if (*e == '<' && e[1] != '<') { const char* t = strchr(e, '>'); if (t) name.append(e, t + 1); }
    auto it = agg.find(name);
    if (it == agg.end()) { order.push_back(name); it = agg.emplace(name, std::make_pair(0, 0.0)).first; }
    it->second.first += 1;
    it->second.second += ms;
  }
  std::string out = "kernel,launches,ms\n";
  for (const auto& n : order) {
    char line[256];
    snprintf(line, sizeof line, "%s,%d,%.4f\n", n.c_str(), agg[n].first, agg[n].second);
    out += line;
  }
  if ((int)out.size() + 1 > cap) return fail(PF_ERR_ARG, "pf_profile_kernels_read: buffer too small (%d needed)", (int)out.size() + 1);
  memcpy(buf, out.c_str(), out.size() + 1);
  h->kp.used = 0;
  h->kp.recs.clear();
  return (int)out.size();
}
int pf_set_option(pf_handle h, const char* name, int value) {
  if (!h || !name) return fail(PF_ERR_ARG, "pf_set_option: null argument");
  if (!strcmp(name, "attn_mma")) { h->use_attn_mma = value != 0; return PF_OK; }
  if (!strcmp(name, "stem_tc")) { h->use_stem_tc = value != 0; return PF_OK; }
  if (!strcmp(name, "phase_conv1")) { h->use_phase = value != 0; return PF_OK; }
  if (!strcmp(name, "attn_split")) { h->use_attn_split = value != 0; return PF_OK; }
  if (!strcmp(name, "decode_only")) { h->decode_only = value != 0; return PF_OK; }
  if (!strcmp(name, "pdl")) { h->use_pdl = value != 0; return PF_OK; }
  if (!strcmp(name, "dw_ln")) { h->use_dwln = value != 0; return PF_OK; }
  if (!strcmp(name, "fork")) { h->use_fork = value != 0; return PF_OK; }
  if (!strcmp(name, "bf16")) { h->bf16 = value != 0; return PF_OK; }
  return fail(PF_ERR_ARG, "pf_set_option: unknown option '%s'", name);
}
int pf_profile_read(pf_handle h, double* out9) {
  if (!h || !out9) return fail(PF_ERR_ARG, "pf_profile_read: null argument");
  for (int i = 0; i < 21; ++i) out9[i] = 0.0;
  FILE* csv = nullptr;
  if (const char* path = getenv("PF_PROFILE_CSV")) {
    csv = fopen(path, "w");
    if (csv) fprintf(csv, "engine_cfg,M,N,K,Cin,KH,stride,groups,ms,algorithmic_tflops\n");
  }
  for (auto& r : h->prof) {
    float ms = 0.f;
    CU(cudaEventSynchronize(r.b));
    CU(cudaEventElapsedTime(&ms, r.a, r.b));
    if (csv) fprintf(csv, "%d,%d,%d,%d,%d,%d,%d,%d,%.4f,%.1f\n", r.cfg, r.M, r.N, r.K, r.Cin, r.KH, r.stride, r.groups, ms, r.flops / (ms * 1e9));
    out9[r.cfg * 3 + 0] += ms;
    out9[r.cfg * 3 + 1] += r.flops;
    out9[r.cfg * 3 + 2] += 1.0;
    h->ev_pool.push_back(r.a);
    h->ev_pool.push_back(r.b);
  }
  if (csv) fclose(csv);
  h->prof.clear();
  return PF_OK;
}

int pf_debug_enable(pf_handle h, int on) {
  if (!h) return fail(PF_ERR_ARG, "null handle");
  h->debug = on != 0;
  h->taps.clear();
  return PF_OK;
}
int pf_debug_count(pf_handle h) { return h ? (int)h->taps.size() : 0; }
const char* pf_debug_name(pf_handle h, int i) { return (h && i >= 0 && i < (int)h->taps.size()) ? h->taps[i].first.c_str() : ""; }
int64_t pf_debug_numel(pf_handle h, const char* name) {
  if (!h || !name) return -1;
  for (auto& t : h->taps) if (t.first == name) return t.second.second;
  return -1;
}
int pf_debug_copy(pf_handle h, const char* name, float* dst, int64_t numel, void* stream) {
  if (!h || !name || !dst) return fail(PF_ERR_ARG, "pf_debug_copy: null argument");
  for (auto& t : h->taps)
    if (t.first == name) {
      if (numel != t.second.second) return fail(PF_ERR_ARG, "pf_debug_copy: '%s' has %lld elements", name, t.second.second);
      CU(cudaMemcpyAsync(dst, t.second.first, numel * 4, cudaMemcpyDeviceToDevice, (cudaStream_t)stream));
      return PF_OK;
    }
  return fail(PF_ERR_ARG, "pf_debug_copy: no tap '%s'", name);
}

#define NCCL_TRY(expr)                                                                                              \
  do {                                                                                                              \
    int r__ = (expr);                                                                                               \
    if (r__ != kNcclSuccess) return fail(PF_ERR_CUDA, "%s: %s", #expr, api.GetErrorString ? api.GetErrorString(r__) : "NCCL error"); \
  } while (0)
int pf_comm_unique_id(void* id128) {
  if (!id128) return fail(PF_ERR_ARG, "pf_comm_unique_id: null argument");
  const NcclApi& api = nccl_api();
  if (api.error) return fail(PF_ERR_CUDA, "%s", api.error);
  static_assert(sizeof(NcclUniqueId) == 128, "ncclUniqueId is 128 bytes");
  NCCL_TRY(api.GetUniqueId((NcclUniqueId*)id128));
  return PF_OK;
}
int pf_comm_create(int device, int rank, int nranks, const void* id128, pf_comm_handle* out) {
  if (!id128 || !out || nranks < 1 || rank < 0 || rank >= nranks) return fail(PF_ERR_ARG, "pf_comm_create: bad argument");
  const NcclApi& api = nccl_api();
  if (api.error) return fail(PF_ERR_CUDA, "%s", api.error);
  CU(cudaSetDevice(device));
  NcclUniqueId id;
  memcpy(&id, id128, sizeof id);
  pf_comm* c = new pf_comm();
  c->device = device; c->rank = rank; c->nranks = nranks;
  const int r = api.CommInitRank(&c->comm, nranks, id, rank);
  if (r != kNcclSuccess) { delete c; return fail(PF_ERR_CUDA, "ncclCommInitRank: %s", api.GetErrorString(r)); }
  *out = c;
  return PF_OK;
}
int pf_comm_destroy(pf_comm_handle c) {
  if (!c) return PF_OK;
  const NcclApi& api = nccl_api();
  cudaSetDevice(c->device);
  if (c->comm && api.CommDestroy) api.CommDestroy(c->comm);
  delete c;
  return PF_OK;
}
int pf_gather(pf_comm_handle c, int root, int count, void* const* dev_ptrs, const int64_t* bytes, const int32_t* peer, void* stream) {
  if (!c || count < 0 || root < 0 || root >= c->nranks || (count > 0 && (!dev_ptrs || !bytes))) return fail(PF_ERR_ARG, "pf_gather: bad argument");
  if (c->rank == root && count > 0 && !peer) return fail(PF_ERR_ARG, "pf_gather: the root needs the source rank of every segment");
  const NcclApi& api = nccl_api();
  CU(cudaSetDevice(c->device));
  if (count == 0) return PF_OK;
  NCCL_TRY(api.GroupStart());
  for (int i = 0; i < count; ++i) {
    int r;
    if (c->rank == root) {
      if (peer[i] < 0 || peer[i] >= c->nranks || peer[i] == root) { api.GroupEnd(); return fail(PF_ERR_ARG, "pf_gather: segment %d comes from rank %d", i, peer[i]); }
      r = api.Recv(dev_ptrs[i], (size_t)bytes[i], kNcclUint8, peer[i], c->comm, (cudaStream_t)stream);
    } else {
      r = api.Send(dev_ptrs[i], (size_t)bytes[i], kNcclUint8, root, c->comm, (cudaStream_t)stream);
    }
    if (r != kNcclSuccess) { api.GroupEnd(); return fail(PF_ERR_CUDA, "ncclSend/Recv: %s", api.GetErrorString(r)); }
  }
  NCCL_TRY(api.GroupEnd());
  return PF_OK;
}

int pf_jpeg_create(int device, int max_threads, pf_jpeg_handle* out) {
  if (!out) return fail(PF_ERR_ARG, "pf_jpeg_create: null argument");
  const NvjpegApi& api = nvjpeg_api();
  if (api.error) return fail(PF_ERR_CUDA, "%s", api.error);
  CU(cudaSetDevice(device));
  pf_jpeg* j = new pf_jpeg();
  j->device = device;
  if (api.CreateSimple(&j->handle) != NVJPEG_STATUS_SUCCESS) { delete j; return fail(PF_ERR_CUDA, "nvjpegCreateSimple failed"); }
  int nt = max_threads > 0 ? max_threads : (int)std::thread::hardware_concurrency() / 2;
  nt = nt < 1 ? 1 : (nt > 32 ? 32 : nt);
  j->workers.resize(nt);
  bool ok = cudaEventCreateWithFlags(&j->start, cudaEventDisableTiming) == cudaSuccess;
  for (auto& w : j->workers) {
    ok = ok && api.StateCreate(j->handle, &w.state) == NVJPEG_STATUS_SUCCESS;
    ok = ok && cudaStreamCreateWithFlags(&w.stream, cudaStreamNonBlocking) == cudaSuccess;
    ok = ok && cudaEventCreateWithFlags(&w.done, cudaEventDisableTiming) == cudaSuccess;
  }
  if (!ok) { pf_jpeg_destroy(j); return fail(PF_ERR_CUDA, "pf_jpeg_create: decoder state / stream creation failed"); }
  *out = j;
  return PF_OK;
}
int pf_jpeg_destroy(pf_jpeg_handle j) {
  if (!j) return PF_OK;
  const NvjpegApi& api = nvjpeg_api();
  cudaSetDevice(j->device);
  for (auto& w : j->workers) {
    if (w.stream) cudaStreamSynchronize(w.stream);
    if (w.state) api.StateDestroy(w.state);
    if (w.stream) cudaStreamDestroy(w.stream);
    if (w.done) cudaEventDestroy(w.done);
  }
  if (j->start) cudaEventDestroy(j->start);
  if (j->handle) api.Destroy(j->handle);
  delete j;
  return PF_OK;
}
int pf_jpeg_info(pf_jpeg_handle j, const uint8_t* data, int64_t length, int32_t* height, int32_t* width) {
  if (!j || !data || length < 4 || !height || !width) return fail(PF_ERR_ARG, "pf_jpeg_info: bad argument");
  const NvjpegApi& api = nvjpeg_api();
  int nc = 0, ws[NVJPEG_MAX_COMPONENT] = {0}, hs[NVJPEG_MAX_COMPONENT] = {0};
  nvjpegChromaSubsampling_t ss;
  if (api.GetImageInfo(j->handle, data, (size_t)length, &nc, &ss, ws, hs) != NVJPEG_STATUS_SUCCESS) return fail(PF_ERR_ARG, "pf_jpeg_info: not a decodable JPEG stream");
  *height = hs[0]; *width = ws[0];
  return PF_OK;
}
int pf_jpeg_decode_batch(pf_jpeg_handle j, int n, const uint8_t* const* data, const int64_t* length, const int32_t* height, const int32_t* width,
                         uint8_t* blob, const int64_t* offset, void* stream) {
  if (!j || n < 1 || !data || !length || !height || !width || !blob || !offset) return fail(PF_ERR_ARG, "pf_jpeg_decode_batch: bad argument");
  const NvjpegApi& api = nvjpeg_api();
  CU(cudaSetDevice(j->device));
  cudaStream_t st = (cudaStream_t)stream;
  CU(cudaEventRecord(j->start, st));
  const int nt = (int)j->workers.size() < n ? (int)j->workers.size() : n;
  std::atomic<int> next{0}, failed{-1};
  auto work = [&](int t) {
    cudaSetDevice(j->device);
    pf_jpeg::Worker& w = j->workers[t];
    cudaStreamWaitEvent(w.stream, j->start, 0);
    for (int i = next.fetch_add(1); i < n; i = next.fetch_add(1)) {
      nvjpegImage_t dst{};
      dst.channel[0] = blob + offset[i];
      dst.pitch[0] = (size_t)width[i] * 3;
      if (api.Decode(j->handle, w.state, data[i], (size_t)length[i], NVJPEG_OUTPUT_BGRI, &dst, w.stream) != NVJPEG_STATUS_SUCCESS) failed.store(i);
    }
    cudaEventRecord(w.done, w.stream);
  };
  std::vector<std::thread> threads;
  for (int t = 1; t < nt; ++t) threads.emplace_back(work, t);
  work(0);
  for (auto& th : threads) th.join();
  for (int t = 0; t < nt; ++t) CU(cudaStreamWaitEvent(st, j->workers[t].done, 0));
  if (failed.load() >= 0) return fail(PF_ERR_ARG, "pf_jpeg_decode_batch: image %d could not be decoded", failed.load());
  return PF_OK;
}

int pf_op_conv_gemm(const float* x, int B, int H, int W, int Cin, const void* whi, const void* wlo, const float* bias, int N, int KH, int KW,
                    int stride, int pad, int in_relu, int act, const float* res, int res_relu, float* y, void* stream) {
  if (!x || !whi || !wlo || !y) return fail(PF_ERR_ARG, "pf_op_conv_gemm: null argument");
  if (KH != KW) return fail(PF_ERR_ARG, "pf_op_conv_gemm: square filters only");
  TRY(configure_current_device());
  cudaStream_t st = (cudaStream_t)stream;
  int dev = 0;
  CU(cudaGetDevice(&dev));
  cudaDeviceProp prop;
  CU(cudaGetDeviceProperties(&prop, dev));
  pf_engine tmp;
  tmp.device = dev;
  tmp.sm_count = prop.multiProcessorCount;
  const int OH = (H + 2 * pad - KH) / stride + 1, OW = (W + 2 * pad - KW) / stride + 1;
  const long long nx = (long long)B * H * W * Cin;
  const long long colb = (long long)B * OH * OW * KH * KW * Cin * 4 + (1 << 20);
  char* scratch = nullptr;
  CU(cudaMalloc(&scratch, nx * 4 + colb + 4096));
  Fwd F{&tmp, Arena{}, st, false, B};
  F.ar.base = scratch; F.ar.cap = nx * 4 + colb + 4096;
  SplitT A = F.salloc((long long)B * H * W, Cin);
  int r = PF_OK;
  {
    cudaError_t le = (split_kernel<<<(unsigned)cdivl(nx, 256), 256, 0, st>>>(x, A.hi, A.lo, nx, in_relu), cudaGetLastError());
    g_launches.fetch_add(1, std::memory_order_relaxed);
    if (le != cudaSuccess) r = fail(PF_ERR_CUDA, "split_kernel: %s", cudaGetErrorString(le));
  }
  GemmW w{(const __nv_bfloat16*)whi, (const __nv_bfloat16*)wlo, bias};
  Fwd::Epi o;
  o.C = y; o.ldc = N; o.act = act; o.res = res; o.ldr = N; o.res_relu = res_relu;
  if (r == PF_OK) {
    if (KH == 3 && stride == 1 && pad == 1 && Cin % 64 == 0) r = F.thalo(A, 0, 0, nullptr, 0, 0, B, H, W, Cin, w, N, 1, 0, o);
    else if (KH == 1 && stride == 1 && pad == 0) r = F.tgemm(A, (long long)B * H * W, Cin, 0, w, N, o);
    else r = F.tconv_gather(A, B, H, W, Cin, KH, stride, pad, w, N, o);
  }
  cudaError_t se = cudaStreamSynchronize(st);
  cudaFree(scratch);
  if (r != PF_OK) return r;
  if (se != cudaSuccess) return fail(PF_ERR_CUDA, "pf_op_conv_gemm: %s", cudaGetErrorString(se));
  return PF_OK;
}
static int op_tma(pf_tma_op* op, void* stream, bool bf16) {
  if (!op || !op->a_hi || !op->a_lo || !op->w_hi || !op->w_lo) return fail(PF_ERR_ARG, "pf_op_tma: null argument");
  const pf_tma_op& q = *op;
  if (q.mode != MODE_GEMM && q.mode != MODE_HALO) return fail(PF_ERR_ARG, "pf_op_tma: mode %d", q.mode);
  if (!q.C && !q.s_hi) return fail(PF_ERR_ARG, "pf_op_tma: no output (C and S are both NULL)");
  if (!q.s_hi != !q.s_lo || !q.a2_hi != !q.a2_lo) return fail(PF_ERR_ARG, "pf_op_tma: a split pair needs both planes");
  if (q.bias_mode < 0 || q.bias_mode > 2 || q.act < 0 || q.act > 2) return fail(PF_ERR_ARG, "pf_op_tma: bias_mode %d / act %d", q.bias_mode, q.act);
  if (q.groups < 1 || q.groups > 2 || q.N < 1) return fail(PF_ERR_ARG, "pf_op_tma: groups %d, N %d", q.groups, q.N);
  if (q.npred != 0 && q.npred != q.groups) return fail(PF_ERR_ARG, "pf_op_tma: npred must be 0 or groups");
  if (q.mode == MODE_GEMM && (q.groups != 1 || q.a2_hi || q.phase4 || q.npred || q.M < 1 || q.M > INT32_MAX))
    return fail(PF_ERR_ARG, "pf_op_tma: GEMM mode runs one group of 1..2^31-1 rows without A2, phase4 or prediction tail");
  if (q.mode == MODE_HALO && (q.B < 1 || q.H < 1 || q.W < 1)) return fail(PF_ERR_ARG, "pf_op_tma: image size %dx%dx%d", q.B, q.H, q.W);
  TRY(configure_current_device());
  int dev = 0;
  CU(cudaGetDevice(&dev));
  cudaDeviceProp prop;
  CU(cudaGetDeviceProperties(&prop, dev));
  pf_engine tmp;
  tmp.device = dev;
  tmp.sm_count = prop.multiProcessorCount;
  tmp.bf16 = bf16;
  Fwd F{&tmp, Arena{}, (cudaStream_t)stream, false, q.B};
  if (q.force_sched < 0 || q.force_sched > 2 || (q.force_sched && q.mode != MODE_GEMM)) return fail(PF_ERR_ARG, "pf_op_tma: force_sched %d", q.force_sched);
  F.force_bn = q.force_bn; F.force_kb = q.force_kb; F.force_sched = q.force_sched;
  const SplitT A{(__nv_bfloat16*)q.a_hi, (__nv_bfloat16*)q.a_lo, q.lda};
  const SplitT A2{(__nv_bfloat16*)q.a2_hi, (__nv_bfloat16*)q.a2_lo, q.lda2};
  const GemmW w{(const __nv_bfloat16*)q.w_hi, (const __nv_bfloat16*)q.w_lo, q.bias};
  Fwd::Epi o;
  o.C = q.C; o.ldc = q.ldc; o.c_coff = q.c_coff; o.c_gcoff = q.c_gcoff;
  o.S = SplitT{(__nv_bfloat16*)q.s_hi, (__nv_bfloat16*)q.s_lo, q.lds}; o.s_coff = q.s_coff; o.s_gcoff = q.s_gcoff; o.split_relu = q.split_relu;
  o.act = q.act; o.gamma = q.gamma;
  o.res = q.res; o.ldr = q.ldr; o.r_coff = q.r_coff; o.r_gcoff = q.r_gcoff; o.res_relu = q.res_relu;
  o.res2 = q.res2; o.ldr2 = q.ldr2; o.r2_coff = q.r2_coff; o.r2_gcoff = q.r2_gcoff;
  o.bias_mode = q.bias_mode; o.phase4 = q.phase4;
  PredTail pt[2];
  for (int g = 0; g < q.npred; ++g) {
    const pf_tma_pred& s = q.pred[g];
    if (!s.w || !s.b || !s.out || !(s.mode == 1 ? s.nc == 2 : (s.mode == 2 && s.nc == 1))) return fail(PF_ERR_ARG, "pf_op_tma: prediction tail %d", g);
    pt[g] = PredTail{s.w, s.b, s.out, s.nc, s.mode};
  }
  op->picked_bn = op->picked_kb = op->picked_sched = 0;
  const int r = q.mode == MODE_GEMM ? F.tgemm(A, q.M, q.K, q.a_c0, w, q.N, o)
                                    : F.thalo(A, q.a_c0, q.a_gc, q.a2_hi ? &A2 : nullptr, q.c_split, q.a2_c0, q.B, q.H, q.W, q.Cin, w, q.N, q.groups,
                                              q.bias_gstride, o, q.npred ? pt : nullptr);
  if (r == PF_OK) { op->picked_bn = F.picked_bn; op->picked_kb = F.picked_kb; op->picked_sched = F.picked_sched; }
  return r;
}
int pf_op_tma(pf_tma_op* op, void* stream) { return op_tma(op, stream, false); }
int pf_op_tma_bf16(pf_tma_op* op, void* stream) { return op_tma(op, stream, true); }
int pf_op_conv1_ring(const void* c_hi, const void* c_lo, int B, int H, int W, const float* wf, const float* bias, float* out,
                     const float* pg_w, const float* pg_b, float* pg_out, const float* pl_w, const float* pl_b, float* pl_out, void* stream) {
  if (!c_hi || !c_lo || !wf || !bias) return fail(PF_ERR_ARG, "pf_op_conv1_ring: null argument");
  const bool tail = pg_w || pg_b || pg_out || pl_w || pl_b || pl_out;
  if (tail && !(pg_w && pg_b && pg_out && pl_w && pl_b && pl_out)) return fail(PF_ERR_ARG, "pf_op_conv1_ring: the prediction tail needs all six pointers");
  if (!out && !tail) return fail(PF_ERR_ARG, "pf_op_conv1_ring: no output");
  if (B < 1 || H < 2 || W < 2) return fail(PF_ERR_ARG, "pf_op_conv1_ring: needs B >= 1 and H, W >= 2 (got %dx%dx%d)", B, H, W);
  TRY(configure_current_device());
  const dim3 grid((unsigned)cdiv(conv1_ring_count(2 * H, 2 * W), kRingPx), (unsigned)B);
  LAUNCHED((conv1_ring_kernel<<<grid, 256, kRingSmem, (cudaStream_t)stream>>>((const __nv_bfloat16*)c_hi, (const __nv_bfloat16*)c_lo, H, W, wf, bias, out,
                                                                             pg_w, pg_b, pg_out, pl_w, pl_b, pl_out), cudaGetLastError()));
  return PF_OK;
}
int pf_tma_pick_tile(int mode, int64_t M, int N, int K, int sm_count, int* bn, int* kb) {
  if (!bn || !kb || (mode != MODE_GEMM && mode != MODE_HALO) || N < 1 || K < 1 || sm_count < 1) return fail(PF_ERR_ARG, "pf_tma_pick_tile: bad argument");
  tma_pick_tile(mode, M, N, K, sm_count, *bn, *kb);
  return PF_OK;
}
int pf_camera_fields(int device, const pf_camera* cams, int n, float* up, float* lat, void* stream) {
  if (!cams || n < 1 || (!up && !lat)) return fail(PF_ERR_ARG, "pf_camera_fields: bad argument");
  CU(cudaSetDevice(device));
  for (int i0 = 0; i0 < n; i0 += kCamChunk) {
    const int m = n - i0 < kCamChunk ? n - i0 : kCamChunk;
    CamBatch b{};
    long long max_q = 1;
    for (int i = 0; i < m; ++i) {
      const pf_camera& c = cams[i0 + i];
      if (c.height < 1 || c.width < 1 || !(c.focal_rel != 0.0)) return fail(PF_ERR_ARG, "pf_camera_fields: image %d: size %dx%d, focal %g", i0 + i, c.height, c.width, c.focal_rel);
      if ((c.up_offset & 1) != 0) return fail(PF_ERR_ARG, "pf_camera_fields: up_offset must be even (8-byte stores)");
      CamImage& o = b.im[i];
      o.H = c.height; o.W = c.width;
      o.f = c.focal_rel * c.height;
      o.cx = (c.cx_rel + 0.5) * c.width; o.cy = (c.cy_rel + 0.5) * c.height;
      o.sr = sin(c.roll); o.cr = cos(c.roll); o.se = sin(c.elevation); o.ce = cos(c.elevation);
      o.sgn = c.elevation > 0 ? 1.0 : (c.elevation < 0 ? -1.0 : 0.0);
      o.up_off = c.up_offset; o.lat_off = c.lat_offset;
      const long long qd = (long long)c.height * ((c.width + 3) / 4);
      if (qd > max_q) max_q = qd;
    }
    const dim3 grid((unsigned)cdivl(max_q, 256), (unsigned)m);
    LAUNCHED((camera_fields_kernel<<<grid, 256, 0, (cudaStream_t)stream>>>(b, up, lat), cudaGetLastError()));
  }
  return PF_OK;
}

int pf_pano_views(int device, const uint8_t* pano, int pano_h, int pano_w, const pf_pano_view* views, int n, uint8_t* im, float* ntheta,
                  float* nphi, float* up, float* lat, float* xy, double* offset, int32_t* status, void* stream) {
  if (!pano || !views || n < 1) return fail(PF_ERR_ARG, "pf_pano_views: null panorama / views or n < 1");
  if (pano_h < 2 || pano_w < 2) return fail(PF_ERR_ARG, "pf_pano_views: panorama of %dx%d (needs at least 2x2)", pano_h, pano_w);
  if (!im && !ntheta && !nphi && !up && !lat && !xy && !offset && !status) return fail(PF_ERR_ARG, "pf_pano_views: no output");
  for (int i = 0; i < n; ++i) {
    const pf_pano_view& c = views[i];
    if (c.height < 1 || c.width < 1) return fail(PF_ERR_ARG, "pf_pano_views: view %d has size %dx%d", i, c.height, c.width);
    if (!std::isfinite(c.f) || !(c.f > 0.0) || !std::isfinite(c.xi) || !std::isfinite(c.az) || !std::isfinite(c.el) || !std::isfinite(c.roll))
      return fail(PF_ERR_ARG, "pf_pano_views: view %d: f must be finite and > 0, xi and the angles finite (f %g, xi %g)", i, c.f, c.xi);
    if (c.im_offset < 0 || c.field_offset < 0) return fail(PF_ERR_ARG, "pf_pano_views: view %d has a negative offset", i);
  }
  CU(cudaSetDevice(device));
  PanoMap m{};
  m.Hp = pano_h; m.Wp = pano_w;
  m.ax = (M_PI - -M_PI) / ((pano_w - 1.0) - 0);
  m.bx = M_PI - m.ax * (pano_w - 1.0);
  m.iax = 1.0 / m.ax;
  m.ay = (-M_PI / 2.0 - M_PI / 2.0) / ((pano_h - 1.0) - 0);
  m.by = M_PI / 2.0 - m.ay * 0;
  m.iay = 1.0 / m.ay;
  auto rad = [](double deg) { return deg * M_PI / 180; };
  for (int i0 = 0; i0 < n; i0 += kPanoChunk) {
    const int cnt = n - i0 < kPanoChunk ? n - i0 : kPanoChunk;
    PanoBatch b{};
    long long max_px = 1;
    for (int i = 0; i < cnt; ++i) {
      const pf_pano_view& c = views[i0 + i];
      PanoView& o = b.v[i];
      o.H = c.height; o.W = c.width;
      o.f = c.f; o.xi = c.xi; o.one_m_xi2 = 1 - c.xi * c.xi;
      o.u0 = c.width / 2.0; o.v0 = c.height / 2.0;
      const double ce = cos(rad(c.el)), se = sin(rad(c.el)), ca = cos(rad(c.az)), sa = sin(rad(c.az)), cr = cos(rad(c.roll)), sr = sin(rad(c.roll));
      const double rel[9] = {1.0, 0.0, 0.0, 0.0, ce, -se, 0.0, se, ce};
      const double raz[9] = {ca, 0.0, sa, 0.0, 1.0, 0.0, -sa, 0.0, ca};
      const double rroll[9] = {cr, -sr, 0.0, sr, cr, 0.0, 0.0, 0.0, 1.0};
      memcpy(o.rel, rel, sizeof rel); memcpy(o.raz, raz, sizeof raz); memcpy(o.rroll, rroll, sizeof rroll);
      const double fmin = sqrt(-(1 - c.xi * c.xi) * ((1 - o.u0) * (1 - o.u0) + (1 - o.v0) * (1 - o.v0))) * 1.0001;
      o.masked = c.f < fmin;
      const double r = sqrt(-(c.f * c.f) / (1 - c.xi * c.xi));
      o.r2 = r * r;
      o.ci0 = nearbyint(c.height / 2.0); o.ci1 = nearbyint(c.width / 2.0);
      o.im_off = c.im_offset; o.fld_off = c.field_offset;
      const long long px = (long long)c.height * c.width;
      if (px > max_px) max_px = px;
    }
    const dim3 grid((unsigned)cdivl(max_px, (long long)kPanoThreads * kPanoPix) + 1, (unsigned)cnt);
    LAUNCHED((pano_views_kernel<<<grid, kPanoThreads, 0, (cudaStream_t)stream>>>(b, m, pano, im, ntheta, nphi, up, lat, xy, offset, status, i0),
              cudaGetLastError()));
  }
  return PF_OK;
}

static int upload_table(const ResampleTable& t, int** bounds, int** coeffs) {
  CU(cudaMalloc(bounds, t.bounds.size() * 4));
  CU(cudaMalloc(coeffs, t.coeffs.size() * 4));
  CU(cudaMemcpy(*bounds, t.bounds.data(), t.bounds.size() * 4, cudaMemcpyHostToDevice));
  CU(cudaMemcpy(*coeffs, t.coeffs.data(), t.coeffs.size() * 4, cudaMemcpyHostToDevice));
  return PF_OK;
}
int pf_op_resize_u8(const uint8_t* img, int H, int W, int new_h, int new_w, uint8_t* out, void* stream) {
  if (!img || !out || H < 1 || W < 1 || new_h < 1 || new_w < 1) return fail(PF_ERR_ARG, "pf_op_resize_u8: bad argument");
  cudaStream_t st = (cudaStream_t)stream;
  if (H == new_h && W == new_w) {
    CU(cudaMemcpyAsync(out, img, (size_t)H * W * 3, cudaMemcpyDeviceToDevice, st));
    return PF_OK;
  }
  ResampleTable tx = make_resample_table(W, new_w), ty = make_resample_table(H, new_h);
  int *bx = nullptr, *cx = nullptr, *by = nullptr, *cy = nullptr;
  unsigned char* tmp = nullptr;
  int r = upload_table(tx, &bx, &cx);
  if (r == PF_OK) r = upload_table(ty, &by, &cy);
  if (r == PF_OK && cudaMalloc(&tmp, (size_t)H * new_w * 3) != cudaSuccess) r = fail(PF_ERR_CUDA, "pf_op_resize_u8: cudaMalloc");
  if (r == PF_OK) {
    cudaError_t le = (resize_u8_h_kernel<<<(unsigned)cdivl((long long)H * new_w, 256), 256, 0, st>>>(img, H, W, new_w, bx, cx, tx.ksize, tmp), cudaGetLastError());
    if (le == cudaSuccess) le = (resize_u8_v_kernel<<<(unsigned)cdivl((long long)new_h * new_w, 256), 256, 0, st>>>(tmp, H, new_w, new_h, by, cy, ty.ksize, out), cudaGetLastError());
    g_launches.fetch_add(2, std::memory_order_relaxed);
    if (le == cudaSuccess) le = cudaStreamSynchronize(st);
    if (le != cudaSuccess) r = fail(PF_ERR_CUDA, "pf_op_resize_u8: %s", cudaGetErrorString(le));
  }
  cudaFree(bx); cudaFree(cx); cudaFree(by); cudaFree(cy); cudaFree(tmp);
  return r;
}
int pf_op_resize_f32(const float* img, int H, int W, int C, int new_h, int new_w, float* out, void* stream) {
  if (!img || !out || H < 1 || W < 1 || C < 1 || new_h < 1 || new_w < 1) return fail(PF_ERR_ARG, "pf_op_resize_f32: bad argument");
  LAUNCHED((resize_f32_kernel<<<(unsigned)cdivl((long long)new_h * new_w * C, 256), 256, 0, (cudaStream_t)stream>>>(img, H, W, C, new_h, new_w, out), cudaGetLastError()));
  return PF_OK;
}
int pf_op_argmax_decode(const float* logits, float* field, int B, int HW, int NC, int is_gravity, void* stream) {
  if (!logits || !field || B < 1 || HW < 1 || NC < 1) return fail(PF_ERR_ARG, "pf_op_argmax_decode: bad argument");
  LAUNCHED((argmax_decode_kernel<<<(unsigned)cdivl((long long)B * HW, 256), 256, 0, (cudaStream_t)stream>>>(logits, field, B, HW, NC, is_gravity), cudaGetLastError()));
  return PF_OK;
}
int pf_op_pred_argmax_decode(const float* feat, int ld, int coff, const float* w, const float* bias, float* field, int B, int HW, int NC, int is_gravity,
                             void* stream) {
  if (!feat || !w || !bias || !field || B < 1 || HW < 1 || NC < 1 || NC > 256 || (ld & 3) || (coff & 3)) return fail(PF_ERR_ARG, "pf_op_pred_argmax_decode: bad argument");
  LAUNCHED((pred_argmax_decode_kernel<<<ew_grid((long long)B * HW * 4), 256, NC * 37 * 4, (cudaStream_t)stream>>>(feat, ld, coff, w, bias, field, B, HW, NC, is_gravity),
            cudaGetLastError()));
  return PF_OK;
}
int pf_op_postprocess(const float* vec, const float* lat, int n, const int32_t* height, const int32_t* width, float* gravity_original,
                      const int64_t* gravity_original_offset, float* latitude_original, const int64_t* latitude_original_offset, int lat_is_sin,
                      void* stream) {
  if (!vec || !lat || n < 1 || !height || !width || !gravity_original || !gravity_original_offset || !latitude_original || !latitude_original_offset)
    return fail(PF_ERR_ARG, "pf_op_postprocess: bad argument");
  return pf_op_postprocess_sized(vec, lat, n, kNet, kNet, height, width, gravity_original, gravity_original_offset, latitude_original, latitude_original_offset,
                                 lat_is_sin, stream);
}
int pf_op_postprocess_sized(const float* vec, const float* lat, int n, int net_h, int net_w, const int32_t* height, const int32_t* width, float* gravity_original,
                            const int64_t* gravity_original_offset, float* latitude_original, const int64_t* latitude_original_offset, int lat_is_sin,
                            void* stream) {
  if (!vec || !lat || n < 1 || !height || !width || !gravity_original || !gravity_original_offset || !latitude_original || !latitude_original_offset)
    return fail(PF_ERR_ARG, "pf_op_postprocess: bad argument");
  if (!net_size_ok(net_h, net_w)) return fail(PF_ERR_ARG, "pf_op_postprocess: unsupported working size %dx%d", net_h, net_w);
  TRY(configure_current_device());
  PostImage* d_post = nullptr;
  CU(cudaMalloc(&d_post, n * sizeof(PostImage)));
  int r = launch_postprocess(vec, lat, n, net_h, net_w, height, width, gravity_original_offset, latitude_original_offset, gravity_original, latitude_original,
                             lat_is_sin, d_post, (cudaStream_t)stream);
  cudaError_t se = cudaStreamSynchronize((cudaStream_t)stream);
  cudaFree(d_post);
  if (r == PF_OK && se != cudaSuccess) r = fail(PF_ERR_CUDA, "pf_op_postprocess: %s", cudaGetErrorString(se));
  return r;
}

int pf_op_fill_stream(float* dst, int64_t numel, float value, void* stream) {
  if (!dst || numel < 4 || (numel & 3) || ((uintptr_t)dst & 15)) return fail(PF_ERR_ARG, "pf_op_fill_stream: bad argument");
  LAUNCHED((fill_stream_kernel<<<132 * 16, 256, 0, (cudaStream_t)stream>>>(reinterpret_cast<float4*>(dst), numel / 4, value), cudaGetLastError()));
  return PF_OK;
}
int pf_op_layernorm(const float* x, float* y, int64_t rows, int C, const float* w, const float* b, float eps, void* stream) {
  LAUNCHED(layernorm_launch(x, y, rows, C, w, b, eps, (cudaStream_t)stream));
  return PF_OK;
}
int pf_op_attention(const float* q, const float* kv, float* out, int B, int N, int C, int heads, void* stream) {
  TRY(configure_current_device());
  if (C != heads * kAttnD) return fail(PF_ERR_ARG, "pf_op_attention: head_dim must be 64");
  LAUNCHED(attention_launch(q, kv, out, B, N, C, heads, (cudaStream_t)stream));
  return PF_OK;
}
int pf_op_attention_mma(const float* q, const float* kv, float* out, int B, int N, int C, int heads, void* stream) {
  TRY(configure_current_device());
  if (C != heads * kAmD) return fail(PF_ERR_ARG, "pf_op_attention_mma: head_dim must be 64");
  LAUNCHED(attention_mma_launch(q, kv, out, B, N, C, heads, (cudaStream_t)stream));
  return PF_OK;
}
static int op_attention_tc(const float* q, const float* kv, float* out, int B, int N, int C, int heads, void* stream, int np, int nkv = kAmKeys) {
  if (!q || !kv || !out || C != heads * kAmD) return fail(PF_ERR_ARG, "pf_op_attention_tc: head_dim must be 64");
  if (B < 1 || N < 1 || nkv < 1 || nkv > kAmMaxKeys) return fail(PF_ERR_ARG, "pf_op_attention_tc: B %d, N %d, %d keys (1..%d)", B, N, nkv, kAmMaxKeys);
  TRY(configure_current_device());
  cudaStream_t st = (cudaStream_t)stream;
  int dev = 0;
  CU(cudaGetDevice(&dev));
  cudaDeviceProp prop;
  CU(cudaGetDeviceProperties(&prop, dev));
  pf_engine tmp;
  tmp.device = dev;
  tmp.sm_count = prop.multiProcessorCount;
  const long long nq = (long long)B * N * C, nkve = (long long)B * nkv * 2 * C;
  char* scratch = nullptr;
  CU(cudaMalloc(&scratch, (2 * nq + nkve) * 4 + 8192));
  Fwd F{&tmp, Arena{}, st, false, B};
  F.ar.base = scratch; F.ar.cap = (2 * nq + nkve) * 4 + 8192;
  SplitT qs = F.salloc((long long)B * N, C), kvs = F.salloc((long long)B * nkv, 2 * C), as = F.salloc((long long)B * N, C);
  int r = PF_OK;
  cudaError_t le = (split_kernel<<<(unsigned)cdivl(nq, 256), 256, 0, st>>>(q, qs.hi, qs.lo, nq, 0), cudaGetLastError());
  if (le == cudaSuccess) le = (split_kernel<<<(unsigned)cdivl(nkve, 256), 256, 0, st>>>(kv, kvs.hi, kvs.lo, nkve, 0), cudaGetLastError());
  if (le != cudaSuccess) r = fail(PF_ERR_CUDA, "split_kernel: %s", cudaGetErrorString(le));
  if (r == PF_OK) {
    le = attention_mma_launch(nullptr, nullptr, nullptr, B, N, C, heads, st, as, qs, kvs, np, nkv);
    if (le != cudaSuccess) r = fail(PF_ERR_CUDA, "attention_mma_launch: %s", cudaGetErrorString(le));
  }
  if (r == PF_OK) {
    le = (merge_split_kernel<<<(unsigned)cdivl(nq, 256), 256, 0, st>>>(as.hi, as.lo, out, nq), cudaGetLastError());
    if (le != cudaSuccess) r = fail(PF_ERR_CUDA, "merge_split_kernel: %s", cudaGetErrorString(le));
  }
  cudaError_t se = cudaStreamSynchronize(st);
  cudaFree(scratch);
  if (r == PF_OK && se != cudaSuccess) r = fail(PF_ERR_CUDA, "pf_op_attention_tc: %s", cudaGetErrorString(se));
  return r;
}
int pf_op_attention_tc(const float* q, const float* kv, float* out, int B, int N, int C, int heads, void* stream) {
  return op_attention_tc(q, kv, out, B, N, C, heads, stream, 3);
}
int pf_op_attention_tc_bf16(const float* q, const float* kv, float* out, int B, int N, int C, int heads, void* stream) {
  return op_attention_tc(q, kv, out, B, N, C, heads, stream, 1);
}
int pf_op_attention_tc_keys(const float* q, const float* kv, float* out, int B, int N, int NKV, int C, int heads, int bf16, void* stream) {
  return op_attention_tc(q, kv, out, B, N, C, heads, stream, bf16 ? 1 : 3, NKV);
}
int pf_op_dwconv3x3_gelu(const float* x, float* y, int B, int H, int W, int C, const float* w, const float* bias, void* stream) {
  if (C % 4) return fail(PF_ERR_ARG, "C %% 4");
  LAUNCHED(launch_pdl(dwconv3x3_gelu_kernel, dim3(ew_grid((long long)B * ((H + 1) / 2) * ((W + PF_DW3_PX - 1) / PF_DW3_PX) * (C / 4))), dim3(256), 0, (cudaStream_t)stream, x, y, B, H, W, C, w, bias, nullptr, nullptr));
  return PF_OK;
}
int pf_op_dwconv7x7(const float* x, float* y, int B, int H, int W, int C, const float* w, const float* bias, void* stream) {
  if (C % 4) return fail(PF_ERR_ARG, "C %% 4");
  LAUNCHED(launch_pdl(dwconv7x7_kernel, dim3(ew_grid((long long)B * ((H + 1) / 2) * ((W + PF_DW7_PX - 1) / PF_DW7_PX) * (C / 4))), dim3(256), 0, (cudaStream_t)stream, x, y, B, H, W, C, w, bias));
  return PF_OK;
}
int pf_op_upsample2x(const float* x, float* y, int B, int H, int W, int C, void* stream) {
  if (C % 4) return fail(PF_ERR_ARG, "C %% 4");
  LAUNCHED(launch_pdl(upsample2x_kernel, dim3(ew_grid(upsample2x_threads(B, H, W, C))), dim3(256), 0, (cudaStream_t)stream, x, C, 0, y, C, 0, B, H, W, C, nullptr, nullptr));
  return PF_OK;
}
int pf_op_preprocess(const uint8_t* img, int H, int W, const float* mean3, const float* std3, float* y, void* stream) {
  return pf_op_preprocess_sized(img, H, W, kNet, kNet, mean3, std3, y, stream);
}
int pf_op_preprocess_sized(const uint8_t* img, int H, int W, int net_h, int net_w, const float* mean3, const float* std3, float* y, void* stream) {
  if (!img || !mean3 || !std3 || !y || H < 1 || W < 1) return fail(PF_ERR_ARG, "pf_op_preprocess: bad argument");
  if (!net_size_ok(net_h, net_w)) return fail(PF_ERR_ARG, "pf_op_preprocess: unsupported working size %dx%d", net_h, net_w);
  TRY(configure_current_device());
  ResampleTable tx = make_resample_table(W, net_w), ty = make_resample_table(H, net_h);
  const int max_rows = pre_max_smem_rows(net_w);
  if (ty.ksize + 1 > max_rows) return fail(PF_ERR_ARG, "image too tall");
  int *bx, *cx, *by, *cy;
  PreImage* d;
  CU(cudaMalloc(&bx, tx.bounds.size() * 4)); CU(cudaMalloc(&cx, tx.coeffs.size() * 4));
  CU(cudaMalloc(&by, ty.bounds.size() * 4)); CU(cudaMalloc(&cy, ty.coeffs.size() * 4));
  CU(cudaMalloc(&d, sizeof(PreImage)));
  CU(cudaMemcpy(bx, tx.bounds.data(), tx.bounds.size() * 4, cudaMemcpyHostToDevice));
  CU(cudaMemcpy(cx, tx.coeffs.data(), tx.coeffs.size() * 4, cudaMemcpyHostToDevice));
  CU(cudaMemcpy(by, ty.bounds.data(), ty.bounds.size() * 4, cudaMemcpyHostToDevice));
  CU(cudaMemcpy(cy, ty.coeffs.data(), ty.coeffs.size() * 4, cudaMemcpyHostToDevice));
  PreImage pi{0, H, W, tx.ksize, ty.ksize, bx, cx, by, cy};
  CU(cudaMemcpy(d, &pi, sizeof pi, cudaMemcpyHostToDevice));
  int rows = pre_rows_needed(H, net_h);
  if (rows > max_rows) rows = max_rows;
  const int smem = rows * net_w * 3;
  LAUNCHED((preprocess_kernel<<<dim3(net_h / kPreRows, 1), net_w, smem, (cudaStream_t)stream>>>(img, d, y, mean3[0], mean3[1], mean3[2], std3[0], std3[1], std3[2], rows,
                                                                                                 net_h, net_w),
            cudaGetLastError()));
  CU(cudaStreamSynchronize((cudaStream_t)stream));
  cudaFree(bx); cudaFree(cx); cudaFree(by); cudaFree(cy); cudaFree(d);
  return PF_OK;
}

}
```

### perspectivefields_b200/csrc/tma_host.cuh

```cuda
#pragma once
#include <cuda.h>
#include <cuda_runtime.h>

#include <cstdlib>
#include <string>

#include "gemm_tma.cuh"

namespace pf {

typedef CUresult (*PFN_tensorMapEncodeTiled)(CUtensorMap*, CUtensorMapDataType, cuuint32_t, void*, const cuuint64_t*, const cuuint64_t*,
                                             const cuuint32_t*, const cuuint32_t*, CUtensorMapInterleave, CUtensorMapSwizzle,
                                             CUtensorMapL2promotion, CUtensorMapFloatOOBfill);

inline PFN_tensorMapEncodeTiled tma_encoder() {
  static PFN_tensorMapEncodeTiled fn = nullptr;
  if (!fn) {
    void* p = nullptr;
    cudaDriverEntryPointQueryResult q;
    if (cudaGetDriverEntryPoint("cuTensorMapEncodeTiled", &p, cudaEnableDefault, &q) == cudaSuccess && q == cudaDriverEntryPointSuccess)
      fn = (PFN_tensorMapEncodeTiled)p;
  }
  return fn;
}

inline const char* tma_map_2d(CUtensorMap* m, const void* base, long long cols, long long rows, long long ld, int box_rows, int kb) {
  PFN_tensorMapEncodeTiled enc = tma_encoder();
  if (!enc) return "cuTensorMapEncodeTiled entry point not available";
  cuuint64_t dims[2] = {(cuuint64_t)cols, (cuuint64_t)rows};
  cuuint64_t strides[1] = {(cuuint64_t)ld * 2};
  cuuint32_t box[2] = {(cuuint32_t)kb, (cuuint32_t)box_rows};
  cuuint32_t es[2] = {1, 1};
  if (((uintptr_t)base & 15) || (strides[0] & 15) || box_rows < 1 || box_rows > 256) return "tma_map_2d: alignment / box";
  CUresult r = enc(m, CU_TENSOR_MAP_DATA_TYPE_BFLOAT16, 2, const_cast<void*>(base), dims, strides, box, es, CU_TENSOR_MAP_INTERLEAVE_NONE,
                   kb == 32 ? CU_TENSOR_MAP_SWIZZLE_64B : CU_TENSOR_MAP_SWIZZLE_128B, CU_TENSOR_MAP_L2_PROMOTION_L2_128B,
                   CU_TENSOR_MAP_FLOAT_OOB_FILL_NONE);
  return r == CUDA_SUCCESS ? nullptr : "cuTensorMapEncodeTiled (2d) failed";
}

inline const char* tma_map_halo(CUtensorMap* m, const void* base, int B, int H, int W, int ld) {
  PFN_tensorMapEncodeTiled enc = tma_encoder();
  if (!enc) return "cuTensorMapEncodeTiled entry point not available";
  cuuint64_t dims[4] = {(cuuint64_t)ld, (cuuint64_t)W, (cuuint64_t)H, (cuuint64_t)B};
  cuuint64_t strides[3] = {(cuuint64_t)ld * 2, (cuuint64_t)W * ld * 2, (cuuint64_t)H * W * ld * 2};
  cuuint32_t box[4] = {64, (cuuint32_t)kHtHaloW, (cuuint32_t)kHtHaloH, 1};
  cuuint32_t es[4] = {1, 1, 1, 1};
  if (((uintptr_t)base & 15) || (strides[0] & 15)) return "tma_map_halo: alignment";
  CUresult r = enc(m, CU_TENSOR_MAP_DATA_TYPE_BFLOAT16, 4, const_cast<void*>(base), dims, strides, box, es, CU_TENSOR_MAP_INTERLEAVE_NONE,
                   CU_TENSOR_MAP_SWIZZLE_128B, CU_TENSOR_MAP_L2_PROMOTION_L2_128B, CU_TENSOR_MAP_FLOAT_OOB_FILL_NONE);
  return r == CUDA_SUCCESS ? nullptr : "cuTensorMapEncodeTiled (halo) failed";
}

inline int tma_pick_bn(int N, int mode) {
  const int tiles = cdiv(N, 256);
  int bn = cdiv(cdiv(N, tiles), 32) * 32;
  if (mode == MODE_HALO) bn = bn <= 32 ? 32 : (bn <= 64 ? 64 : (bn <= 128 ? 128 : 256));
  return bn;
}

inline int tma_pick_bn_gemm(long long M, int N, int K, int sm_count) {
  const int base = tma_pick_bn(N, MODE_GEMM);
  const long long mt = cdivl(M, 128);
  if (mt * cdiv(N, base) * 4 > 3LL * sm_count) return base;
  int best = base;
  double best_cost = 1e30;
  for (int bn = base; bn >= 32; bn -= 32) {
    const long long tiles = mt * cdiv(N, bn);
    const double waves = (double)cdivl(tiles, sm_count);
    const double mma = 3.0 * bn, load = 1.6 * (128 + bn);
    const double cost = waves * ((K / 16) * (mma > load ? mma : load) + 3000.0);
    if (cost < best_cost - 1e-9) { best_cost = cost; best = bn; }
  }
  return best;
}

inline int tma_pick_kb(int bn, int K, int mode) {
  const int lim = mode == MODE_HALO ? 128 : 64;
  return (bn <= lim && K % 64 == 0) ? 64 : 32;
}

inline void tma_pick_tile(int mode, long long M, int N, int K, int sm_count, int& bn, int& kb) {
  bn = mode == MODE_GEMM ? tma_pick_bn_gemm(M, N, K, sm_count) : tma_pick_bn(N, mode);
  kb = tma_pick_kb(bn, K, mode);
}

constexpr int kPingPongKMax = 512;
inline bool tma_pick_pingpong(long long M, int N, int K, int bn, int sm_count) {
  return K <= kPingPongKMax && cdivl(M, 64) * cdiv(N, bn) >= 2LL * sm_count;
}

struct PredTail { const float* w; const float* b; float* out; int nc, mode; };

template <int BN, int MODE, int KB, bool PP = false, int NP = 3>
inline cudaError_t gemm_tma_launch_bn(const TmaMaps& maps, const TmaGemmParams& p, int sm_count, cudaStream_t st, const PredTail* pred) {
  using Cfg = TmaCfg<BN, MODE, KB, PP, NP>;
  const int tiles_x = MODE == MODE_HALO ? cdiv(p.W, kHtTileW) : 0, tiles_y = MODE == MODE_HALO ? cdiv(p.H, kHtTileH) : 0;
  const long long m_tiles = MODE == MODE_GEMM ? cdiv(p.M, Cfg::kTileM) : (long long)p.B * tiles_x * tiles_y;
  const long long total = m_tiles * cdiv(p.N, BN) * p.groups;
  const unsigned grid = (unsigned)(total < sm_count ? total : sm_count);
  if (MODE == MODE_HALO && ((p.Cin == 64 && 9 * (64 / KB) <= Cfg::kStages && (p.groups > 1 || cdiv(p.N, BN) > 1)) || pred)) {
    cudaError_t last = cudaSuccess;
    for (int g = 0; g < p.groups; ++g)
      for (int nt = 0; nt < cdiv(p.N, BN); ++nt) {
        TmaGemmParams q = p;
        q.groups = 1;
        q.a_c0 = p.a_c0 + g * p.a_gc;
        q.bias = p.bias ? p.bias + (long long)g * p.bias_gstride : nullptr;
        q.c_coff = p.c_coff + g * p.c_gcoff; q.s_coff = p.s_coff + g * p.s_gcoff;
        q.r_coff = p.r_coff + g * p.r_gcoff; q.r2_coff = p.r2_coff + g * p.r2_gcoff;
        q.b_row0 = g * p.N;
        if (pred) { q.pred_w = pred[g].w; q.pred_b = pred[g].b; q.pred_out = pred[g].out; q.pred_nc = pred[g].nc; q.pred_mode = pred[g].mode; }
        if (cdiv(p.N, BN) > 1) return cudaErrorInvalidValue;
        const unsigned gr = (unsigned)(m_tiles < sm_count ? m_tiles : sm_count);
        last = launch_pdl(gemm_tma_kernel<BN, MODE, KB, false, NP>, dim3(gr), dim3(kTmaThreads), Cfg::kSmemBytes, st, maps, q, tiles_x, tiles_y);
        if (last != cudaSuccess) return last;
      }
    return last;
  }
  return launch_pdl(gemm_tma_kernel<BN, MODE, KB, PP, NP>, dim3(grid), dim3(kTmaThreads), Cfg::kSmemBytes, st, maps, p, tiles_x, tiles_y);
}

#define PF_TMA_VARIANTS(X)                                                                                                  \
  X(256, MODE_GEMM, 32) X(224, MODE_GEMM, 32) X(192, MODE_GEMM, 32) X(160, MODE_GEMM, 32) X(128, MODE_GEMM, 32) X(96, MODE_GEMM, 32) \
  X(64, MODE_GEMM, 32) X(32, MODE_GEMM, 32) X(64, MODE_GEMM, 64) X(32, MODE_GEMM, 64)                                        \
  X(256, MODE_HALO, 32) X(128, MODE_HALO, 64) X(64, MODE_HALO, 64) X(32, MODE_HALO, 64)
#define PF_TMA_PINGPONG_VARIANTS(X)                                                                                         \
  X(256, 32) X(224, 32) X(192, 32) X(160, 32) X(128, 32) X(96, 32) X(64, 32) X(32, 32) X(64, 64) X(32, 64)

template <int NP>
inline cudaError_t gemm_tma_configure_np() {
  cudaError_t e = cudaSuccess;
#define PF_TMA_CFG(BN_, MODE_, KB_)                                                                                          \
  if (e == cudaSuccess) e = cudaFuncSetAttribute(gemm_tma_kernel<BN_, MODE_, KB_, false, NP>, cudaFuncAttributeMaxDynamicSharedMemorySize, TmaCfg<BN_, MODE_, KB_, false, NP>::kSmemBytes);
  PF_TMA_VARIANTS(PF_TMA_CFG)
#undef PF_TMA_CFG
#define PF_TMA_CFG_PP(BN_, KB_)                                                                                               \
  if (e == cudaSuccess) e = cudaFuncSetAttribute(gemm_tma_kernel<BN_, MODE_GEMM, KB_, true, NP>, cudaFuncAttributeMaxDynamicSharedMemorySize, TmaCfg<BN_, MODE_GEMM, KB_, true, NP>::kSmemBytes);
  PF_TMA_PINGPONG_VARIANTS(PF_TMA_CFG_PP)
#undef PF_TMA_CFG_PP
  return e;
}
inline cudaError_t gemm_tma_configure_device(int np) {
  return np == 1 ? gemm_tma_configure_np<1>() : (np == 3 ? gemm_tma_configure_np<3>() : cudaErrorInvalidValue);
}

template <int NP>
inline int tma_stages_np(int mode, int bn, int kb, bool pp) {
#define PF_TMA_NS(BN_, MODE_, KB_) if (!pp && mode == MODE_ && bn == BN_ && kb == KB_) return TmaCfg<BN_, MODE_, KB_, false, NP>::kStages;
  PF_TMA_VARIANTS(PF_TMA_NS)
#undef PF_TMA_NS
#define PF_TMA_NS_PP(BN_, KB_) if (pp && mode == MODE_GEMM && bn == BN_ && kb == KB_) return TmaCfg<BN_, MODE_GEMM, KB_, true, NP>::kStages;
  PF_TMA_PINGPONG_VARIANTS(PF_TMA_NS_PP)
#undef PF_TMA_NS_PP
  return 0;
}
inline int tma_stages(int mode, int bn, int kb, bool pp, int np) {
  return np == 1 ? tma_stages_np<1>(mode, bn, kb, pp) : (np == 3 ? tma_stages_np<3>(mode, bn, kb, pp) : 0);
}

inline const char* gemm_tma_check(int mode, const TmaGemmParams& p, int bn, int kb, bool pred, bool pp, int np) {
  const int ns = tma_stages(mode, bn, kb, pp, np);
  if (!ns) return pp ? "no ping-pong engine instantiation for this (mode, bn, kb)" : "no engine instantiation for this (mode, bn, kb)";
  if (mode == MODE_GEMM) return p.K % kb ? "GEMM mode: K must be a multiple of the K step" : nullptr;
  if (p.phase4 && (p.N != 128 || bn != 128)) return "phase4 needs N = 128 in one 128-wide tile";
  if (pred && bn != (p.phase4 ? 128 : 32)) return "the fused prediction tail needs N = 32 (phase4: 128) in one tile";
  const bool resident = p.Cin == 64 && 9 * (64 / kb) <= ns;
  if ((resident || pred) && cdiv(p.N, bn) > 1) return "resident weights (Cin = 64) and the prediction tail need one N tile per launch";
  return nullptr;
}

template <int NP>
inline cudaError_t gemm_tma_launch_np(int mode, const TmaMaps& maps, const TmaGemmParams& p, int bn, int kb, bool pp, int sm_count, cudaStream_t st,
                                      const PredTail* pred) {
#define PF_TMA_CASE(BN_, MODE_, KB_) if (!pp && mode == MODE_ && bn == BN_ && kb == KB_) return gemm_tma_launch_bn<BN_, MODE_, KB_, false, NP>(maps, p, sm_count, st, pred);
  PF_TMA_VARIANTS(PF_TMA_CASE)
#undef PF_TMA_CASE
#define PF_TMA_CASE_PP(BN_, KB_) if (pp && mode == MODE_GEMM && bn == BN_ && kb == KB_) return gemm_tma_launch_bn<BN_, MODE_GEMM, KB_, true, NP>(maps, p, sm_count, st, pred);
  PF_TMA_PINGPONG_VARIANTS(PF_TMA_CASE_PP)
#undef PF_TMA_CASE_PP
  return cudaErrorInvalidValue;
}
inline cudaError_t gemm_tma_launch(int mode, const TmaMaps& maps, const TmaGemmParams& p, int bn, int kb, bool pp, int np, int sm_count, cudaStream_t st,
                                   const PredTail* pred = nullptr) {
  if (np == 1) return gemm_tma_launch_np<1>(mode, maps, p, bn, kb, pp, sm_count, st, pred);
  if (np == 3) return gemm_tma_launch_np<3>(mode, maps, p, bn, kb, pp, sm_count, st, pred);
  return cudaErrorInvalidValue;
}

}
```

Before: 616.1.

## Add ping-pong schedule for halo-mode implicit-GEMM conv with 128x128 tiles

```diff
diff --git a/perspectivefields_b200/csrc/gemm_tma.cuh b/perspectivefields_b200/csrc/gemm_tma.cuh
--- a/perspectivefields_b200/csrc/gemm_tma.cuh
+++ b/perspectivefields_b200/csrc/gemm_tma.cuh
@@ -31,10 +31,11 @@
 template <int BN, int MODE, int KB, bool PP = false, int NP = 3> struct TmaCfg {
   static_assert(KB == 32 || KB == 64, "KB");
   static_assert(BN % 32 == 0 && BN <= 256, "BN");
-  static_assert(!PP || MODE == MODE_GEMM, "the ping-pong schedule is a GEMM-mode schedule");
+  static_assert(!PP || MODE == MODE_GEMM || (BN == 128 && KB == 64), "the halo-mode ping-pong schedule runs 128 x 128 tiles, KB = 64");
   static_assert(NP == 1 || NP == 3, "NP");
   static constexpr int kPlanes = NP == 3 ? 2 : 1;
-  static constexpr int kTileM = PP ? 64 : 128;
+  static constexpr int kHalves = PP && MODE == MODE_HALO ? 2 : 1;
+  static constexpr int kTileM = PP && MODE == MODE_GEMM ? 64 : 128;
   static constexpr int kBPlane = BN * KB * 2;
   static constexpr int kAPlane = kTileM * KB * 2;
   static constexpr int kStage = (MODE == MODE_GEMM ? kPlanes * kAPlane : 0) + kPlanes * kBPlane;
@@ -75,6 +76,8 @@
   constexpr int NS = Cfg::kStages;
   constexpr int SPC = 9 * (64 / KB);
   constexpr int kConsumerWarps = PP ? 4 : 8;
+  constexpr int kHalves = Cfg::kHalves;
+  constexpr int kHalfA = 8 * kHtHaloW * 128;
   extern __shared__ unsigned char smem_dyn[];
   const uint32_t raw = smem_u32(smem_dyn);
   const uint32_t sbase = (raw + 1023u) & ~1023u;
@@ -95,7 +98,7 @@
   const int total_tiles = m_tiles * n_tiles * p.groups;
   const int nchunks = MODE == MODE_HALO ? p.Cin / 64 : 0;
   const int nk = MODE == MODE_GEMM ? p.K / KB : nchunks * SPC;
-  const bool b_resident = MODE == MODE_HALO && nchunks == 1 && SPC <= NS;
+  const bool b_resident = !PP && MODE == MODE_HALO && nchunks == 1 && SPC <= NS;
 
   if (tid == 0) {
     tma_prefetch_desc(&maps.a_hi); tma_prefetch_desc(&maps.b_hi);
@@ -173,15 +176,16 @@
   const int wt = tid & 127;
   float* stage = reinterpret_cast<float*>(sm + (acc_base - sbase)) + wg * 64 * Cfg::kAccPitch;
   const int erow = wt & 63, eh = wt >> 6;
-  const int r = PP ? erow : wg * 64 + erow;
+  const int r1 = PP ? erow : wg * 64 + erow;
   constexpr int kTileStep = PP ? 2 : 1;
-  float acc[BN / 2];
+  float acc[kHalves * BN / 2];
   int it = 0, ita = 0;
   for (int tl = PP ? wg : 0, tile = blockIdx.x + tl * gridDim.x; tile < total_tiles; tile += kTileStep * gridDim.x, tl += kTileStep) {
     int mt, g, n0;
     decode(tile, mt, g, n0);
     if (PP) {
       it = tl * nk;
+      if (MODE == MODE_HALO) ita = tl * nchunks;
       if (tl > 0) mbar_wait(order_b(wg ^ 1), ((tl - 1) >> 1) & 1);
     }
     int prev_s = -1, prev_buf = -1;
@@ -196,7 +200,7 @@
         const int tap = KB == 32 ? (u >> 1) : u, ky = tap / 3, kx = tap - ky * 3;
         buf = ita & 1;
         if (u == 0) mbar_wait(full_a(buf), (ita >> 1) & 1);
-        a_hi = a_base + buf * Cfg::kABuf + ((ky + 8 * wg) * kHtHaloW + kx) * 128 + (KB == 32 ? (u & 1) * 64 : 0);
+        a_hi = a_base + buf * Cfg::kABuf + ((ky + (PP ? 0 : 8 * wg)) * kHtHaloW + kx) * 128 + (KB == 32 ? (u & 1) * 64 : 0);
         a_lo = a_hi + kHtPlaneBytes;
         chunk_end = u == SPC - 1;
       } else {
@@ -208,6 +212,7 @@
       const uint32_t b_hi = ring + sb * Cfg::kStage + (MODE == MODE_GEMM ? Cfg::kPlanes * Cfg::kAPlane : 0);
       const uint64_t dah = MODE == MODE_HALO ? ht_a_desc(a_hi) : wgmma_tile_desc<KB>(a_hi);
       const uint64_t dbh = wgmma_tile_desc<KB>(b_hi);
+      constexpr uint64_t kHalfDesc = kHalfA >> 4;
       wgmma_fence();
       if (kLo) {
         const uint64_t dal = MODE == MODE_HALO ? ht_a_desc(a_lo) : wgmma_tile_desc<KB>(a_lo);
@@ -215,13 +220,18 @@
 #pragma unroll
         for (int kk = 0; kk < KB / 16; ++kk) {
           const uint32_t first = (kc | kk) ? 1u : 0u;
-          wgmma_bf16<BN>(acc, dal + 2 * kk, dbh + 2 * kk, first);
-          wgmma_bf16<BN>(acc, dah + 2 * kk, dbl + 2 * kk, 1u);
-          wgmma_bf16<BN>(acc, dah + 2 * kk, dbh + 2 * kk, 1u);
+#pragma unroll
+          for (int h = 0; h < kHalves; ++h) wgmma_bf16<BN>(acc + h * (BN / 2), dal + h * kHalfDesc + 2 * kk, dbh + 2 * kk, first);
+#pragma unroll
+          for (int h = 0; h < kHalves; ++h) wgmma_bf16<BN>(acc + h * (BN / 2), dah + h * kHalfDesc + 2 * kk, dbl + 2 * kk, 1u);
+#pragma unroll
+          for (int h = 0; h < kHalves; ++h) wgmma_bf16<BN>(acc + h * (BN / 2), dah + h * kHalfDesc + 2 * kk, dbh + 2 * kk, 1u);
         }
       } else {
 #pragma unroll
-        for (int kk = 0; kk < KB / 16; ++kk) wgmma_bf16<BN>(acc, dah + 2 * kk, dbh + 2 * kk, (kc | kk) ? 1u : 0u);
+        for (int kk = 0; kk < KB / 16; ++kk)
+#pragma unroll
+          for (int h = 0; h < kHalves; ++h) wgmma_bf16<BN>(acc + h * (BN / 2), dah + h * kHalfDesc + 2 * kk, dbh + 2 * kk, (kc | kk) ? 1u : 0u);
       }
       wgmma_commit();
       wgmma_wait<1>();
@@ -241,205 +251,215 @@
       if (MODE == MODE_HALO && prev_buf >= 0) mbar_arrive(empty_a(prev_buf));
     }
 
-    long long m;
-    bool valid;
-    int cls_off = 0;
-    int bimg = 0, oy = 0, ox = 0;
-    if (MODE == MODE_GEMM) {
-      m = (long long)mt * Cfg::kTileM + r;
-      valid = m < p.M;
-    } else {
-      const int tx = mt % tiles_x, ty = (mt / tiles_x) % tiles_y;
-      bimg = mt / (tiles_x * tiles_y);
-      oy = ty * kHtTileH + (r >> 3); ox = tx * kHtTileW + (r & 7);
-      valid = oy < p.H && ox < p.W;
-      m = ((long long)bimg * p.H + oy) * p.W + ox;
-      if (p.bias_mode == 2) {
-        const int ry = oy == 0 ? 0 : (oy == p.H - 1 ? 2 : 1);
-        const int rx = ox == 0 ? 0 : (ox == p.W - 1 ? 2 : 1);
-        cls_off = (ry * 3 + rx) * p.N;
-      }
-    }
-    const float* __restrict__ bias = p.bias ? p.bias + (long long)g * p.bias_gstride : nullptr;
-    const int frow = (wt >> 5) * 16 + (lane >> 2), fcol = 2 * (lane & 3);
-#pragma unroll
-    for (int rd = 0; rd < (BN + 63) / 64; ++rd) {
-      named_bar_sync(1 + wg, 128);
-#pragma unroll
-      for (int jb = 0; jb < 8; ++jb) {
-        const int cb = rd * 8 + jb;
-        if (cb < BN / 8) {
-          float* d0 = stage + frow * Cfg::kAccPitch + jb * 8 + fcol;
-          *reinterpret_cast<float2*>(d0) = make_float2(acc[4 * cb], acc[4 * cb + 1]);
-          *reinterpret_cast<float2*>(d0 + 8 * Cfg::kAccPitch) = make_float2(acc[4 * cb + 2], acc[4 * cb + 3]);
-        }
-      }
-      named_bar_sync(1 + wg, 128);
-      const int ch = 2 * rd + eh;
-      const bool ph4 = MODE == MODE_HALO && BN == 128 && p.phase4;
-      const bool staged_split = p.Shi && !ph4;
-      float o[32];
-      if (ch < BN / 32) {
-        const int nb = n0 + ch * 32;
-        const long long mo = ph4 ? ((long long)bimg * 2 * p.H + 2 * oy + (ch >> 1)) * (2 * p.W) + 2 * ox + (ch & 1) : m;
-        const int nbo = ph4 ? 0 : nb;
-        const bool chunk_ok = nb < p.N;
-        const float* srow = stage + erow * Cfg::kAccPitch + eh * 32;
-#pragma unroll
-        for (int j = 0; j < 32; j += 4) {
-          const float4 t = *reinterpret_cast<const float4*>(srow + j);
-          o[j] = t.x; o[j + 1] = t.y; o[j + 2] = t.z; o[j + 3] = t.w;
-        }
-        if (valid && chunk_ok) {
-          if (p.bias_mode) {
-#pragma unroll
-            for (int j = 0; j < 32; j += 4) {
-              const float4 bv = __ldg(reinterpret_cast<const float4*>(bias + cls_off + nb + j));
-              o[j] += bv.x; o[j + 1] += bv.y; o[j + 2] += bv.z; o[j + 3] += bv.w;
-            }
-          }
-          if (p.act == 1) {
-#pragma unroll
-            for (int j = 0; j < 32; ++j) o[j] = fmaxf(o[j], 0.f);
-          } else if (p.act == 2) {
-#pragma unroll
-            for (int j = 0; j < 32; ++j) o[j] = gelu_erf(o[j]);
-          }
-          if (p.gamma) {
-#pragma unroll
-            for (int j = 0; j < 32; j += 4) {
-              const float4 gv = __ldg(reinterpret_cast<const float4*>(p.gamma + nb + j));
-              o[j] *= gv.x; o[j + 1] *= gv.y; o[j + 2] *= gv.z; o[j + 3] *= gv.w;
-            }
-          }
-          if (p.res) {
-            const float* rp = p.res + m * p.ldr + p.r_coff + g * p.r_gcoff + nb;
-#pragma unroll
-            for (int j = 0; j < 32; j += 4) {
-              float4 rv = *reinterpret_cast<const float4*>(rp + j);
-              if (p.res_relu) { rv.x = fmaxf(rv.x, 0.f); rv.y = fmaxf(rv.y, 0.f); rv.z = fmaxf(rv.z, 0.f); rv.w = fmaxf(rv.w, 0.f); }
-              o[j] += rv.x; o[j + 1] += rv.y; o[j + 2] += rv.z; o[j + 3] += rv.w;
-            }
-          }
-          if (p.res2) {
-            const float* rp = p.res2 + m * p.ldr2 + p.r2_coff + g * p.r2_gcoff + nb;
-#pragma unroll
-            for (int j = 0; j < 32; j += 4) {
-              const float4 rv = *reinterpret_cast<const float4*>(rp + j);
-              o[j] += rv.x; o[j + 1] += rv.y; o[j + 2] += rv.z; o[j + 3] += rv.w;
-            }
-          }
-          if (MODE == MODE_HALO && (BN == 32 || BN == 128) && p.pred_w) {
-            float v0 = __ldg(p.pred_b), v1 = p.pred_nc > 1 ? __ldg(p.pred_b + 1) : 0.f;
-#pragma unroll
-            for (int j = 0; j < 32; j += 4) {
-              const float4 w0 = __ldg(reinterpret_cast<const float4*>(p.pred_w + j));
-              v0 = fmaf(o[j], w0.x, v0); v0 = fmaf(o[j + 1], w0.y, v0); v0 = fmaf(o[j + 2], w0.z, v0); v0 = fmaf(o[j + 3], w0.w, v0);
-              if (p.pred_nc > 1) {
-                const float4 w1 = __ldg(reinterpret_cast<const float4*>(p.pred_w + 32 + j));
-                v1 = fmaf(o[j], w1.x, v1); v1 = fmaf(o[j + 1], w1.y, v1); v1 = fmaf(o[j + 2], w1.z, v1); v1 = fmaf(o[j + 3], w1.w, v1);
-              }
-            }
-            const long long HWl = (long long)p.H * p.W * (ph4 ? 4 : 1);
-            const long long bi = mo / HWl, pix = mo - bi * HWl;
-            float* po = p.pred_out + bi * p.pred_nc * HWl + pix;
-            if (p.pred_mode == 1) {
-              const float nrm = fmaxf(sqrtf(v0 * v0 + v1 * v1), 1e-12f);
-              po[0] = v0 / nrm; po[HWl] = v1 / nrm;
+#pragma unroll
+    for (int hf = 0; hf < kHalves; ++hf) {
+      const int row0 = kHalves == 2 ? hf * 64 : (PP ? 0 : wg * 64);
+      const int r = kHalves == 2 ? row0 + erow : r1;
+      const float* ah = acc + hf * (BN / 2);
+      long long m;
+      bool valid;
+      int cls_off = 0;
+      int bimg = 0, oy = 0, ox = 0;
+      if (MODE == MODE_GEMM) {
+        m = (long long)mt * Cfg::kTileM + r;
+        valid = m < p.M;
+      } else {
+        const int tx = mt % tiles_x, ty = (mt / tiles_x) % tiles_y;
+        bimg = mt / (tiles_x * tiles_y);
+        oy = ty * kHtTileH + (r >> 3); ox = tx * kHtTileW + (r & 7);
+        valid = oy < p.H && ox < p.W;
+        m = ((long long)bimg * p.H + oy) * p.W + ox;
+        if (p.bias_mode == 2) {
+          const int ry = oy == 0 ? 0 : (oy == p.H - 1 ? 2 : 1);
+          const int rx = ox == 0 ? 0 : (ox == p.W - 1 ? 2 : 1);
+          cls_off = (ry * 3 + rx) * p.N;
+        }
+      }
+      const float* __restrict__ bias = p.bias ? p.bias + (long long)g * p.bias_gstride : nullptr;
+      const int frow = (wt >> 5) * 16 + (lane >> 2), fcol = 2 * (lane & 3);
+  #pragma unroll
+      for (int rd = 0; rd < (BN + 63) / 64; ++rd) {
+        named_bar_sync(1 + wg, 128);
+  #pragma unroll
+        for (int jb = 0; jb < 8; ++jb) {
+          const int cb = rd * 8 + jb;
+          if (cb < BN / 8) {
+            float* d0 = stage + frow * Cfg::kAccPitch + jb * 8 + fcol;
+            *reinterpret_cast<float2*>(d0) = make_float2(ah[4 * cb], ah[4 * cb + 1]);
+            *reinterpret_cast<float2*>(d0 + 8 * Cfg::kAccPitch) = make_float2(ah[4 * cb + 2], ah[4 * cb + 3]);
+          }
+        }
+        named_bar_sync(1 + wg, 128);
+        const int ch = 2 * rd + eh;
+        const bool ph4 = MODE == MODE_HALO && BN == 128 && p.phase4;
+        const bool staged_split = p.Shi && !ph4;
+        float o[32];
+        if (ch < BN / 32) {
+          const int nb = n0 + ch * 32;
+          const long long mo = ph4 ? ((long long)bimg * 2 * p.H + 2 * oy + (ch >> 1)) * (2 * p.W) + 2 * ox + (ch & 1) : m;
+          const int nbo = ph4 ? 0 : nb;
+          const bool chunk_ok = nb < p.N;
+          const float* srow = stage + erow * Cfg::kAccPitch + eh * 32;
+  #pragma unroll
+          for (int j = 0; j < 32; j += 4) {
+            const float4 t = *reinterpret_cast<const float4*>(srow + j);
+            o[j] = t.x; o[j + 1] = t.y; o[j + 2] = t.z; o[j + 3] = t.w;
+          }
+          if (valid && chunk_ok) {
+            if (p.bias_mode) {
+  #pragma unroll
+              for (int j = 0; j < 32; j += 4) {
+                const float4 bv = __ldg(reinterpret_cast<const float4*>(bias + cls_off + nb + j));
+                o[j] += bv.x; o[j + 1] += bv.y; o[j + 2] += bv.z; o[j + 3] += bv.w;
+              }
+            }
+            if (p.act == 1) {
+  #pragma unroll
+              for (int j = 0; j < 32; ++j) o[j] = fmaxf(o[j], 0.f);
+            } else if (p.act == 2) {
+  #pragma unroll
+              for (int j = 0; j < 32; ++j) o[j] = gelu_erf(o[j]);
+            }
+            if (p.gamma) {
+  #pragma unroll
+              for (int j = 0; j < 32; j += 4) {
+                const float4 gv = __ldg(reinterpret_cast<const float4*>(p.gamma + nb + j));
+                o[j] *= gv.x; o[j + 1] *= gv.y; o[j + 2] *= gv.z; o[j + 3] *= gv.w;
+              }
+            }
+            if (p.res) {
+              const float* rp = p.res + m * p.ldr + p.r_coff + g * p.r_gcoff + nb;
+  #pragma unroll
+              for (int j = 0; j < 32; j += 4) {
+                float4 rv = *reinterpret_cast<const float4*>(rp + j);
+                if (p.res_relu) { rv.x = fmaxf(rv.x, 0.f); rv.y = fmaxf(rv.y, 0.f); rv.z = fmaxf(rv.z, 0.f); rv.w = fmaxf(rv.w, 0.f); }
+                o[j] += rv.x; o[j + 1] += rv.y; o[j + 2] += rv.z; o[j + 3] += rv.w;
+              }
+            }
+            if (p.res2) {
+              const float* rp = p.res2 + m * p.ldr2 + p.r2_coff + g * p.r2_gcoff + nb;
+  #pragma unroll
+              for (int j = 0; j < 32; j += 4) {
+                const float4 rv = *reinterpret_cast<const float4*>(rp + j);
+                o[j] += rv.x; o[j + 1] += rv.y; o[j + 2] += rv.z; o[j + 3] += rv.w;
+              }
+            }
+            if (MODE == MODE_HALO && (BN == 32 || BN == 128) && p.pred_w) {
+              float v0 = __ldg(p.pred_b), v1 = p.pred_nc > 1 ? __ldg(p.pred_b + 1) : 0.f;
+  #pragma unroll
+              for (int j = 0; j < 32; j += 4) {
+                const float4 w0 = __ldg(reinterpret_cast<const float4*>(p.pred_w + j));
+                v0 = fmaf(o[j], w0.x, v0); v0 = fmaf(o[j + 1], w0.y, v0); v0 = fmaf(o[j + 2], w0.z, v0); v0 = fmaf(o[j + 3], w0.w, v0);
+                if (p.pred_nc > 1) {
+                  const float4 w1 = __ldg(reinterpret_cast<const float4*>(p.pred_w + 32 + j));
+                  v1 = fmaf(o[j], w1.x, v1); v1 = fmaf(o[j + 1], w1.y, v1); v1 = fmaf(o[j + 2], w1.z, v1); v1 = fmaf(o[j + 3], w1.w, v1);
+                }
+              }
+              const long long HWl = (long long)p.H * p.W * (ph4 ? 4 : 1);
+              const long long bi = mo / HWl, pix = mo - bi * HWl;
+              float* po = p.pred_out + bi * p.pred_nc * HWl + pix;
+              if (p.pred_mode == 1) {
+                const float nrm = fmaxf(sqrtf(v0 * v0 + v1 * v1), 1e-12f);
+                po[0] = v0 / nrm; po[HWl] = v1 / nrm;
+              } else {
+                po[0] = fminf(fmaxf(v0, -1.f), 1.f);
+              }
+            }
+          }
+          if (chunk_ok && (p.C || (p.Shi && !staged_split))) {
+            const bool odd = lane & 1;
+            const bool valid_p = __shfl_xor_sync(0xffffffffu, (int)valid, 1) != 0;
+            const long long mo_p = mo + (odd ? -1 : 1) * (ph4 ? 2 : 1);
+            const long long moA = odd ? mo_p : mo, moB = odd ? mo : mo_p;
+            const bool vA = odd ? valid_p : valid, vB = odd ? valid : valid_p;
+            if (p.C) {
+              float* cA = p.C + moA * p.ldc + p.c_coff + g * p.c_gcoff + nbo + (odd ? 4 : 0);
+              float* cB = p.C + moB * p.ldc + p.c_coff + g * p.c_gcoff + nbo + (odd ? 4 : 0);
+  #pragma unroll
+              for (int t = 0; t < 4; ++t) {
+                float k[4], rr[4];
+  #pragma unroll
+                for (int e = 0; e < 4; ++e) {
+                  k[e] = odd ? o[8 * t + 4 + e] : o[8 * t + e];
+                  rr[e] = __shfl_xor_sync(0xffffffffu, odd ? o[8 * t + e] : o[8 * t + 4 + e], 1);
+                }
+                if (vA) *reinterpret_cast<float4*>(cA + 8 * t) = odd ? make_float4(rr[0], rr[1], rr[2], rr[3]) : make_float4(k[0], k[1], k[2], k[3]);
+                if (vB) *reinterpret_cast<float4*>(cB + 8 * t) = odd ? make_float4(k[0], k[1], k[2], k[3]) : make_float4(rr[0], rr[1], rr[2], rr[3]);
+              }
+            }
+            if (p.Shi && !staged_split) {
+              const long long sA = moA * p.lds + p.s_coff + g * p.s_gcoff + nbo + (odd ? 8 : 0);
+              const long long sB = moB * p.lds + p.s_coff + g * p.s_gcoff + nbo + (odd ? 8 : 0);
+  #pragma unroll
+              for (int t = 0; t < 2; ++t) {
+                float k[8], rr[8];
+  #pragma unroll
+                for (int e = 0; e < 8; ++e) {
+                  const float mine = odd ? o[16 * t + 8 + e] : o[16 * t + e], give = odd ? o[16 * t + e] : o[16 * t + 8 + e];
+                  k[e] = p.split_relu ? fmaxf(mine, 0.f) : mine;
+                  rr[e] = __shfl_xor_sync(0xffffffffu, p.split_relu ? fmaxf(give, 0.f) : give, 1);
+                }
+                uint4 kh, kl, rh, rl;
+                split_bf16x2(k[0], k[1], kh.x, kl.x); split_bf16x2(k[2], k[3], kh.y, kl.y);
+                split_bf16x2(k[4], k[5], kh.z, kl.z); split_bf16x2(k[6], k[7], kh.w, kl.w);
+                split_bf16x2(rr[0], rr[1], rh.x, rl.x); split_bf16x2(rr[2], rr[3], rh.y, rl.y);
+                split_bf16x2(rr[4], rr[5], rh.z, rl.z); split_bf16x2(rr[6], rr[7], rh.w, rl.w);
+                if (vA) {
+                  *reinterpret_cast<uint4*>(p.Shi + sA + 16 * t) = odd ? rh : kh;
+                  *reinterpret_cast<uint4*>(p.Slo + sA + 16 * t) = odd ? rl : kl;
+                }
+                if (vB) {
+                  *reinterpret_cast<uint4*>(p.Shi + sB + 16 * t) = odd ? kh : rh;
+                  *reinterpret_cast<uint4*>(p.Slo + sB + 16 * t) = odd ? kl : rl;
+                }
+              }
+            }
+          }
+        }
+        if (staged_split) {
+          named_bar_sync(1 + wg, 128);
+          unsigned char* sS = reinterpret_cast<unsigned char*>(stage);
+          if (ch < BN / 32) {
+  #pragma unroll
+            for (int t = 0; t < 4; ++t) {
+              uint4 h, l;
+              float k[8];
+  #pragma unroll
+              for (int e = 0; e < 8; ++e) k[e] = p.split_relu ? fmaxf(o[8 * t + e], 0.f) : o[8 * t + e];
+              split_bf16x2(k[0], k[1], h.x, l.x); split_bf16x2(k[2], k[3], h.y, l.y);
+              split_bf16x2(k[4], k[5], h.z, l.z); split_bf16x2(k[6], k[7], h.w, l.w);
+              const int off = erow * 128 + (((eh * 4 + t) ^ (erow & 7)) << 4);
+              *reinterpret_cast<uint4*>(sS + off) = h;
+              *reinterpret_cast<uint4*>(sS + 64 * 128 + off) = l;
+            }
+          }
+          named_bar_sync(1 + wg, 128);
+  #pragma unroll
+          for (int i = wt; i < 2 * 64 * 8; i += 128) {
+            const int lo_plane = i >> 9, rr = (i >> 3) & 63, pc = i & 7;
+            const int col = rd * 64 + pc * 8;
+            if (col >= BN || n0 + col >= p.N) continue;
+            long long mr;
+            bool vr;
+            if (MODE == MODE_GEMM) {
+              mr = (long long)mt * Cfg::kTileM + row0 + rr;
+              vr = mr < p.M;
             } else {
-              po[0] = fminf(fmaxf(v0, -1.f), 1.f);
-            }
-          }
-        }
-        if (chunk_ok && (p.C || (p.Shi && !staged_split))) {
-          const bool odd = lane & 1;
-          const bool valid_p = __shfl_xor_sync(0xffffffffu, (int)valid, 1) != 0;
-          const long long mo_p = mo + (odd ? -1 : 1) * (ph4 ? 2 : 1);
-          const long long moA = odd ? mo_p : mo, moB = odd ? mo : mo_p;
-          const bool vA = odd ? valid_p : valid, vB = odd ? valid : valid_p;
-          if (p.C) {
-            float* cA = p.C + moA * p.ldc + p.c_coff + g * p.c_gcoff + nbo + (odd ? 4 : 0);
-            float* cB = p.C + moB * p.ldc + p.c_coff + g * p.c_gcoff + nbo + (odd ? 4 : 0);
-#pragma unroll
-            for (int t = 0; t < 4; ++t) {
-              float k[4], rr[4];
-#pragma unroll
-              for (int e = 0; e < 4; ++e) {
-                k[e] = odd ? o[8 * t + 4 + e] : o[8 * t + e];
-                rr[e] = __shfl_xor_sync(0xffffffffu, odd ? o[8 * t + e] : o[8 * t + 4 + e], 1);
-              }
-              if (vA) *reinterpret_cast<float4*>(cA + 8 * t) = odd ? make_float4(rr[0], rr[1], rr[2], rr[3]) : make_float4(k[0], k[1], k[2], k[3]);
-              if (vB) *reinterpret_cast<float4*>(cB + 8 * t) = odd ? make_float4(k[0], k[1], k[2], k[3]) : make_float4(rr[0], rr[1], rr[2], rr[3]);
-            }
-          }
-          if (p.Shi && !staged_split) {
-            const long long sA = moA * p.lds + p.s_coff + g * p.s_gcoff + nbo + (odd ? 8 : 0);
-            const long long sB = moB * p.lds + p.s_coff + g * p.s_gcoff + nbo + (odd ? 8 : 0);
-#pragma unroll
-            for (int t = 0; t < 2; ++t) {
-              float k[8], rr[8];
-#pragma unroll
-              for (int e = 0; e < 8; ++e) {
-                const float mine = odd ? o[16 * t + 8 + e] : o[16 * t + e], give = odd ? o[16 * t + e] : o[16 * t + 8 + e];
-                k[e] = p.split_relu ? fmaxf(mine, 0.f) : mine;
-                rr[e] = __shfl_xor_sync(0xffffffffu, p.split_relu ? fmaxf(give, 0.f) : give, 1);
-              }
-              uint4 kh, kl, rh, rl;
-              split_bf16x2(k[0], k[1], kh.x, kl.x); split_bf16x2(k[2], k[3], kh.y, kl.y);
-              split_bf16x2(k[4], k[5], kh.z, kl.z); split_bf16x2(k[6], k[7], kh.w, kl.w);
-              split_bf16x2(rr[0], rr[1], rh.x, rl.x); split_bf16x2(rr[2], rr[3], rh.y, rl.y);
-              split_bf16x2(rr[4], rr[5], rh.z, rl.z); split_bf16x2(rr[6], rr[7], rh.w, rl.w);
-              if (vA) {
-                *reinterpret_cast<uint4*>(p.Shi + sA + 16 * t) = odd ? rh : kh;
-                *reinterpret_cast<uint4*>(p.Slo + sA + 16 * t) = odd ? rl : kl;
-              }
-              if (vB) {
-                *reinterpret_cast<uint4*>(p.Shi + sB + 16 * t) = odd ? kh : rh;
-                *reinterpret_cast<uint4*>(p.Slo + sB + 16 * t) = odd ? kl : rl;
-              }
-            }
-          }
-        }
-      }
-      if (staged_split) {
-        named_bar_sync(1 + wg, 128);
-        unsigned char* sS = reinterpret_cast<unsigned char*>(stage);
-        if (ch < BN / 32) {
-#pragma unroll
-          for (int t = 0; t < 4; ++t) {
-            uint4 h, l;
-            float k[8];
-#pragma unroll
-            for (int e = 0; e < 8; ++e) k[e] = p.split_relu ? fmaxf(o[8 * t + e], 0.f) : o[8 * t + e];
-            split_bf16x2(k[0], k[1], h.x, l.x); split_bf16x2(k[2], k[3], h.y, l.y);
-            split_bf16x2(k[4], k[5], h.z, l.z); split_bf16x2(k[6], k[7], h.w, l.w);
-            const int off = erow * 128 + (((eh * 4 + t) ^ (erow & 7)) << 4);
-            *reinterpret_cast<uint4*>(sS + off) = h;
-            *reinterpret_cast<uint4*>(sS + 64 * 128 + off) = l;
-          }
-        }
-        named_bar_sync(1 + wg, 128);
-#pragma unroll
-        for (int i = wt; i < 2 * 64 * 8; i += 128) {
-          const int lo_plane = i >> 9, rr = (i >> 3) & 63, pc = i & 7;
-          const int col = rd * 64 + pc * 8;
-          if (col >= BN || n0 + col >= p.N) continue;
-          long long mr;
-          bool vr;
-          if (MODE == MODE_GEMM) {
-            mr = (long long)mt * Cfg::kTileM + (PP ? 0 : wg * 64) + rr;
-            vr = mr < p.M;
-          } else {
-            const int rt = wg * 64 + rr, tx = mt % tiles_x, ty = (mt / tiles_x) % tiles_y;
-            const int py = ty * kHtTileH + (rt >> 3), px = tx * kHtTileW + (rt & 7);
-            vr = py < p.H && px < p.W;
-            mr = ((long long)bimg * p.H + py) * p.W + px;
-          }
-          if (!vr) continue;
-          const uint4 v = *reinterpret_cast<const uint4*>(sS + lo_plane * 64 * 128 + rr * 128 + ((pc ^ (rr & 7)) << 4));
-          *reinterpret_cast<uint4*>((lo_plane ? p.Slo : p.Shi) + mr * p.lds + p.s_coff + g * p.s_gcoff + n0 + col) = v;
-        }
-      }
+              const int rt = row0 + rr, tx = mt % tiles_x, ty = (mt / tiles_x) % tiles_y;
+              const int py = ty * kHtTileH + (rt >> 3), px = tx * kHtTileW + (rt & 7);
+              vr = py < p.H && px < p.W;
+              mr = ((long long)bimg * p.H + py) * p.W + px;
+            }
+            if (!vr) continue;
+            const uint4 v = *reinterpret_cast<const uint4*>(sS + lo_plane * 64 * 128 + rr * 128 + ((pc ^ (rr & 7)) << 4));
+            *reinterpret_cast<uint4*>((lo_plane ? p.Slo : p.Shi) + mr * p.lds + p.s_coff + g * p.s_gcoff + n0 + col) = v;
+          }
+        }
+      }
+    }
+    if (kHalves == 2) {
+#pragma unroll
+      for (int i = 0; i < kHalves * BN / 2; ++i) acc[i] = 0.f;
     }
   }
 }
diff --git a/perspectivefields_b200/csrc/pf_b200.cu b/perspectivefields_b200/csrc/pf_b200.cu
--- a/perspectivefields_b200/csrc/pf_b200.cu
+++ b/perspectivefields_b200/csrc/pf_b200.cu
@@ -347,9 +347,17 @@
     tma_pick_tile(mode, p.M, p.N, p.K, e->sm_count, bn, kb);
     if (force_bn) { bn = force_bn; kb = tma_pick_kb(bn, p.K, mode); }
     if (force_kb) kb = force_kb;
-    pp = mode == MODE_GEMM && (force_sched ? force_sched == 2 : tma_pick_pingpong(p.M, p.N, p.K, bn, e->sm_count));
+    if (mode == MODE_GEMM) {
+      pp = force_sched ? force_sched == 2 : tma_pick_pingpong(p.M, p.N, p.K, bn, e->sm_count);
+    } else {
+      const long long pp_tiles = (long long)p.B * cdiv(p.H, kHtTileH) * cdiv(p.W, kHtTileW) * cdiv(p.N, 128) * p.groups;
+      pp = force_sched ? force_sched == 3
+                       : !force_bn && tma_pick_halo_pingpong(bn, pp_tiles, e->sm_count) && !gemm_tma_check(mode, p, 128, 64, pred != nullptr, true, np());
+      if (pp && !force_bn) bn = 128;
+      if (pp && !force_kb) kb = 64;
+    }
     if (const char* msg = gemm_tma_check(mode, p, bn, kb, pred != nullptr, pp, np())) return fail(PF_ERR_ARG, "TMA engine, %s (bn %d, kb %d): %s", mode == MODE_GEMM ? "GEMM mode" : "halo mode", bn, kb, msg);
-    picked_bn = bn; picked_kb = kb; picked_sched = mode == MODE_GEMM ? (pp ? 2 : 1) : 0;
+    picked_bn = bn; picked_kb = kb; picked_sched = mode == MODE_GEMM ? (pp ? 2 : 1) : (pp ? 3 : 0);
     return PF_OK;
   }
   int launch_tma(int mode, const TmaMaps& maps, const TmaGemmParams& p, int bn, int kb, bool pp, const PredTail* pred = nullptr) {
@@ -1356,7 +1364,8 @@
   tmp.sm_count = prop.multiProcessorCount;
   tmp.bf16 = bf16;
   Fwd F{&tmp, Arena{}, (cudaStream_t)stream, false, q.B};
-  if (q.force_sched < 0 || q.force_sched > 2 || (q.force_sched && q.mode != MODE_GEMM)) return fail(PF_ERR_ARG, "pf_op_tma: force_sched %d", q.force_sched);
+  if (q.force_sched < 0 || q.force_sched > 3 || (q.force_sched == 2 && q.mode != MODE_GEMM) || (q.force_sched == 3 && q.mode != MODE_HALO))
+    return fail(PF_ERR_ARG, "pf_op_tma: force_sched %d in %s mode", q.force_sched, q.mode == MODE_GEMM ? "GEMM" : "halo");
   F.force_bn = q.force_bn; F.force_kb = q.force_kb; F.force_sched = q.force_sched;
   const SplitT A{(__nv_bfloat16*)q.a_hi, (__nv_bfloat16*)q.a_lo, q.lda};
   const SplitT A2{(__nv_bfloat16*)q.a2_hi, (__nv_bfloat16*)q.a2_lo, q.lda2};
diff --git a/perspectivefields_b200/csrc/tma_host.cuh b/perspectivefields_b200/csrc/tma_host.cuh
--- a/perspectivefields_b200/csrc/tma_host.cuh
+++ b/perspectivefields_b200/csrc/tma_host.cuh
@@ -89,6 +89,8 @@
   return K <= kPingPongKMax && cdivl(M, 64) * cdiv(N, bn) >= 2LL * sm_count;
 }
 
+inline bool tma_pick_halo_pingpong(int bn, long long pp_tiles, int sm_count) { return bn == 256 && pp_tiles >= 4LL * sm_count; }
+
 struct PredTail { const float* w; const float* b; float* out; int nc, mode; };
 
 template <int BN, int MODE, int KB, bool PP = false, int NP = 3>
@@ -98,7 +100,7 @@
   const long long m_tiles = MODE == MODE_GEMM ? cdiv(p.M, Cfg::kTileM) : (long long)p.B * tiles_x * tiles_y;
   const long long total = m_tiles * cdiv(p.N, BN) * p.groups;
   const unsigned grid = (unsigned)(total < sm_count ? total : sm_count);
-  if (MODE == MODE_HALO && ((p.Cin == 64 && 9 * (64 / KB) <= Cfg::kStages && (p.groups > 1 || cdiv(p.N, BN) > 1)) || pred)) {
+  if (MODE == MODE_HALO && !PP && ((p.Cin == 64 && 9 * (64 / KB) <= Cfg::kStages && (p.groups > 1 || cdiv(p.N, BN) > 1)) || pred)) {
     cudaError_t last = cudaSuccess;
     for (int g = 0; g < p.groups; ++g)
       for (int nt = 0; nt < cdiv(p.N, BN); ++nt) {
@@ -127,6 +129,8 @@
 #define PF_TMA_PINGPONG_VARIANTS(X)                                                                                         \
   X(256, 32) X(224, 32) X(192, 32) X(160, 32) X(128, 32) X(96, 32) X(64, 32) X(32, 32) X(64, 64) X(32, 64)
 
+#define PF_TMA_HALO_PINGPONG_VARIANTS(X) X(128, 64)
+
 template <int NP>
 inline cudaError_t gemm_tma_configure_np() {
   cudaError_t e = cudaSuccess;
@@ -138,6 +142,10 @@
   if (e == cudaSuccess) e = cudaFuncSetAttribute(gemm_tma_kernel<BN_, MODE_GEMM, KB_, true, NP>, cudaFuncAttributeMaxDynamicSharedMemorySize, TmaCfg<BN_, MODE_GEMM, KB_, true, NP>::kSmemBytes);
   PF_TMA_PINGPONG_VARIANTS(PF_TMA_CFG_PP)
 #undef PF_TMA_CFG_PP
+#define PF_TMA_CFG_HPP(BN_, KB_)                                                                                              \
+  if (e == cudaSuccess) e = cudaFuncSetAttribute(gemm_tma_kernel<BN_, MODE_HALO, KB_, true, NP>, cudaFuncAttributeMaxDynamicSharedMemorySize, TmaCfg<BN_, MODE_HALO, KB_, true, NP>::kSmemBytes);
+  PF_TMA_HALO_PINGPONG_VARIANTS(PF_TMA_CFG_HPP)
+#undef PF_TMA_CFG_HPP
   return e;
 }
 inline cudaError_t gemm_tma_configure_device(int np) {
@@ -152,6 +160,9 @@
 #define PF_TMA_NS_PP(BN_, KB_) if (pp && mode == MODE_GEMM && bn == BN_ && kb == KB_) return TmaCfg<BN_, MODE_GEMM, KB_, true, NP>::kStages;
   PF_TMA_PINGPONG_VARIANTS(PF_TMA_NS_PP)
 #undef PF_TMA_NS_PP
+#define PF_TMA_NS_HPP(BN_, KB_) if (pp && mode == MODE_HALO && bn == BN_ && kb == KB_) return TmaCfg<BN_, MODE_HALO, KB_, true, NP>::kStages;
+  PF_TMA_HALO_PINGPONG_VARIANTS(PF_TMA_NS_HPP)
+#undef PF_TMA_NS_HPP
   return 0;
 }
 inline int tma_stages(int mode, int bn, int kb, bool pp, int np) {
@@ -162,9 +173,10 @@
   const int ns = tma_stages(mode, bn, kb, pp, np);
   if (!ns) return pp ? "no ping-pong engine instantiation for this (mode, bn, kb)" : "no engine instantiation for this (mode, bn, kb)";
   if (mode == MODE_GEMM) return p.K % kb ? "GEMM mode: K must be a multiple of the K step" : nullptr;
+  const bool resident = p.Cin == 64 && 9 * (64 / kb) <= ns;
+  if (pp && (p.phase4 || pred || resident)) return "the halo-mode ping-pong schedule runs no phase4, prediction tail or resident weights";
   if (p.phase4 && (p.N != 128 || bn != 128)) return "phase4 needs N = 128 in one 128-wide tile";
   if (pred && bn != (p.phase4 ? 128 : 32)) return "the fused prediction tail needs N = 32 (phase4: 128) in one tile";
-  const bool resident = p.Cin == 64 && 9 * (64 / kb) <= ns;
   if ((resident || pred) && cdiv(p.N, bn) > 1) return "resident weights (Cin = 64) and the prediction tail need one N tile per launch";
   return nullptr;
 }
@@ -178,6 +190,9 @@
 #define PF_TMA_CASE_PP(BN_, KB_) if (pp && mode == MODE_GEMM && bn == BN_ && kb == KB_) return gemm_tma_launch_bn<BN_, MODE_GEMM, KB_, true, NP>(maps, p, sm_count, st, pred);
   PF_TMA_PINGPONG_VARIANTS(PF_TMA_CASE_PP)
 #undef PF_TMA_CASE_PP
+#define PF_TMA_CASE_HPP(BN_, KB_) if (pp && mode == MODE_HALO && bn == BN_ && kb == KB_) return gemm_tma_launch_bn<BN_, MODE_HALO, KB_, true, NP>(maps, p, sm_count, st, pred);
+  PF_TMA_HALO_PINGPONG_VARIANTS(PF_TMA_CASE_HPP)
+#undef PF_TMA_CASE_HPP
   return cudaErrorInvalidValue;
 }
 inline cudaError_t gemm_tma_launch(int mode, const TmaMaps& maps, const TmaGemmParams& p, int bn, int kb, bool pp, int np, int sm_count, cudaStream_t st,
```

Result: faster. 625.7 (median of 6 runs) (+1.5%).
